# qinzheng93/GeoTransformer

Hardware: NVIDIA H100
Metric: point-cloud pairs/sec (3DMatch-shape synth) (higher is better)
Workload: dtype f32

## Files before the change

geotransformer_b200/_lib.py:

```python
import ctypes
import os
import threading

import torch

_HERE = os.path.dirname(os.path.abspath(__file__))
LIB_PATH = os.path.join(_HERE, 'libgeob200.so')
_lib = None

c_void_p, c_int64, c_int32, c_float, c_double, c_size_t, c_int = (
    ctypes.c_void_p, ctypes.c_int64, ctypes.c_int32, ctypes.c_float, ctypes.c_double, ctypes.c_size_t, ctypes.c_int)

SIGNATURES = {}


def _sig(name, restype, *argtypes):
    SIGNATURES[name] = (restype, list(argtypes))


P, I64, I32, F, D, SZ = c_void_p, c_int64, c_int32, c_float, c_double, c_size_t
_sig('geob200_last_error', ctypes.c_char_p)
_sig('geob200_launch_count', ctypes.c_uint64)
_sig('geob200_grid_subsample_workspace_bytes', SZ, I64, I64)
_sig('geob200_grid_subsample', c_int, P, I64, P, I64, F, P, P, P, SZ, P)
_sig('geob200_radius_search_workspace_bytes', SZ, I64, I64, I64)
_sig('geob200_radius_search', c_int, P, I64, P, I64, P, P, I64, F, I64, P, P, P, P, SZ, P)

_sig('geob200_neighbor_histogram', c_int, P, I64, I64, I64, I64, P, P)
_sig('geob200_kpconv_workspace_bytes', SZ, I64)
_sig('geob200_kpconv', c_int, P, P, P, P, I64, I64, I64, P, I64, P, P, I64, I64, F, P, P, SZ, P)
_sig('geob200_kpconv_tc_workspace_bytes', SZ, I64, I64, I64)
_sig('geob200_kpconv_tc', c_int, P, P, P, P, I64, I64, I64, P, I64, P, P, I64, I64, F, P, P, SZ, P)
_sig('geob200_set_linear_mode', None, c_int)
_sig('geob200_linear', c_int, P, I64, P, P, P, I64, I64, I64, I64, c_int, P)
_sig('geob200_split_tf32', c_int, P, I64, I64, I64, P, P)
_sig('geob200_linear_batched', c_int, P, I64, I64, P, I64, I64, P, I64, P, I64, I64, I64, I64, I64, I64, c_int, P)
_sig('geob200_group_norm_workspace_bytes', SZ, I64)
_sig('geob200_group_norm', c_int, P, I64, I64, I64, P, P, F, P, c_int, F, P, P, SZ, P)
_sig('geob200_fused_group_norm_workspace_bytes', SZ, I64, I64, I64)
_sig('geob200_linear_group_norm', c_int, P, I64, P, P, I64, I64, I64, I64, P, P, F, P, c_int, F, P, P, P, SZ, P)
_sig('geob200_kpconv_group_norm', c_int, P, P, P, P, I64, I64, I64, P, I64, P, P, I64, I64, F, I64, P, P, F, c_int, F, P, P, P, SZ,
     P, SZ, P)
_sig('geob200_group_norm_batched', c_int, P, I64, I64, I64, P, P, F, P, c_int, F, P, P, SZ, P, I64, P)
_sig('geob200_linear_group_norm_batched', c_int, P, I64, P, P, I64, I64, I64, I64, P, P, F, P, c_int, F, P, P, P, SZ, P, I64, P)
_sig('geob200_maxpool', c_int, P, P, I64, I64, I64, I64, P, P)
_sig('geob200_upsample_concat', c_int, P, P, I64, I64, P, I64, I64, I64, P, P)
_sig('geob200_kpconv_backward_workspace_bytes', SZ, I64, I64, I64, I64, I64)
_sig('geob200_kpconv_backward', c_int, P, P, P, P, I64, I64, I64, P, I64, P, I64, I64, F, P, P, P, P, P, SZ, P)
_sig('geob200_linear_backward_workspace_bytes', SZ, I64, I64, I64, c_int)
_sig('geob200_linear_backward', c_int, P, I64, P, P, I64, I64, I64, P, P, P, P, P, SZ, P)
_sig('geob200_group_norm_backward_batched_workspace_bytes', SZ, I64, I64, I64, I64)
_sig('geob200_group_norm_backward_batched', c_int, P, P, I64, I64, I64, P, F, c_int, F, P, P, P, P, P, P, SZ, P, I64, P)
_sig('geob200_maxpool_backward_batched_workspace_bytes', SZ, I64, I64, I64, I64)
_sig('geob200_maxpool_backward_batched', c_int, P, P, I64, I64, I64, I64, P, I64, P, P, P, P, SZ, P)
_sig('geob200_upsample_concat_backward_workspace_bytes', SZ, I64, I64)
_sig('geob200_upsample_concat_backward', c_int, P, I64, I64, I64, I64, I64, P, P, P, P, SZ, P)
_sig('geob200_point_to_node_partition_batched', c_int, P, P, I64, P, P, I64, P, P, P, P, P, P)
_sig('geob200_gather_rows', c_int, P, I64, I64, P, I64, P, P)
_sig('geob200_knn_partition', c_int, P, I64, P, I64, I64, P, P, P)
_sig('geob200_pairwise_distance', c_int, P, I64, P, I64, I64, c_int, P, P)
_sig('geob200_point_to_node_indices', c_int, P, I64, P, I64, P, P, P)
_sig('geob200_apply_transform', c_int, P, I64, P, P, P)
_sig('geob200_gse_indices_batched', c_int, P, I64, P, F, F, I64, P, P, P)
_sig('geob200_gse_embed_workspace_bytes', SZ, I64, I64)
_sig('geob200_gse_table_bytes', SZ, I64, I64, F, F)
_sig('geob200_gse_table_build', c_int, P, P, P, P, P, I64, I64, F, F, P, SZ, P)
_sig('geob200_gse_embed_table', c_int, P, P, I64, I64, P, SZ, I64, F, F, P, P, P, P, P, P, P)
_sig('geob200_gse_embed_pairs', c_int, P, P, I64, I64, P, P, P, P, P, P, P, P, c_int, P, SZ, P)
_sig('geob200_attention_workspace_bytes', SZ, I64, I64, I64)
_sig('geob200_attention', c_int, P, I64, P, I64, P, I64, P, P, P, I64, I64, I64, I64, P, I64, P, SZ, P)
_sig('geob200_set_attention_tma', c_int, c_int)
_sig('geob200_head_bias', c_int, P, I64, P, I64, I64, I64, P, P)
_sig('geob200_add_layernorm', c_int, P, P, P, P, I64, I64, F, P, P)
_sig('geob200_l2_normalize', c_int, P, I64, I64, P, P)
_sig('geob200_add_layernorm_backward_workspace_bytes', SZ, I64, I64)
_sig('geob200_add_layernorm_backward', c_int, P, P, P, I64, I64, F, P, P, P, P, P, SZ, P)
_sig('geob200_l2_normalize_backward', c_int, P, I64, I64, P, P, P)
_sig('geob200_head_project_backward_workspace_bytes', SZ, I64, I64, I64)
_sig('geob200_head_project_backward', c_int, P, I64, P, P, I64, I64, I64, P, P, P, I64, P, P, P, SZ, P)
_sig('geob200_attention_backward_batched_workspace_bytes', SZ, P, I64, I64)
_sig('geob200_attention_backward_batched', c_int, P, P, I64, I64, I64, I64, I64, I64, I64, I64, I64, I64, P, SZ, P)
_sig('geob200_gse_embed_backward_workspace_bytes', SZ, I64, I64)
_sig('geob200_gse_embed_backward', c_int, P, P, I64, I64, I64, P, SZ, I64, F, F, P, P, P, P, P, P, P, P, P, SZ, P)
_sig('geob200_sinkhorn', c_int, P, P, P, P, I64, I64, I64, F, P, P)
_sig('geob200_sinkhorn_backward_workspace_bytes', SZ, I64, I64, I64)
_sig('geob200_sinkhorn_backward', c_int, P, P, P, P, I64, I64, I64, F, P, P, P, P, SZ, P)
_sig('geob200_superpoint_matching_batched_workspace_bytes', SZ, I64, I64, I64)
_sig('geob200_superpoint_matching_batched', c_int, P, P, I64, P, P, I64, P, I64, c_int, P, P, P, P, SZ, P)
_sig('geob200_gather_patches_batched', c_int, P, I64, I64, P, P, P, P, I64, P, P, P, P, P)
_sig('geob200_patch_scores_batched', c_int, P, P, I64, I64, P, P, P, I64, I64, P, P)
_sig('geob200_patch_scores_backward_batched_workspace_bytes', SZ, I64, I64, I64, I64)
_sig('geob200_patch_scores_backward_batched', c_int, P, P, I64, I64, P, P, P, I64, I64, P, P, P, P, SZ, P)
_sig('geob200_lgr_batched_workspace_bytes', SZ, I64, I64, I64, I64)
_sig('geob200_local_global_registration_batched', c_int, P, P, P, P, P, I64, I64, I64, I64, I64, F, c_int, F, I64, I64, P, P, P, P,
     P, P, I64, P, P, P, P, SZ, P)
_sig('geob200_weighted_procrustes', c_int, P, P, P, I64, I64, F, F, P, P)

_sig('geob200_node_correspondences_batched_workspace_bytes', SZ, I64, I64, I64)
_sig('geob200_node_correspondences_batched', c_int, P, P, P, P, P, P, P, P, I64, P, I64, P, F, P, P, P, P, SZ, P)
_sig('geob200_evaluate_counts', c_int, P, P, I64, P, F, P, P, I64, P, P, P, I64, P, F, P, P, P, I64, c_int, F, F, F, P, P)
_sig('geob200_evaluate_batched', c_int, P, P, P, F, P, P, I64, P, P, P, I64, P, F, P, P, I64, P, I64, P, P, c_int, F, F, F, P, I64,
     P)
_sig('geob200_coarse_matching_loss_batched_workspace_bytes', SZ, I64, I64)
_sig('geob200_coarse_matching_loss_batched', c_int, P, P, I64, I64, P, P, P, P, F, F, F, F, F, F, P, I64, P, SZ, P)
_sig('geob200_fine_matching_loss_batched_workspace_bytes', SZ, I64, I64)
_sig('geob200_fine_matching_loss_batched', c_int, P, P, P, P, P, P, I64, I64, I64, P, D, P, P, I64, P, SZ, P)
_sig('geob200_coarse_matching_loss_backward_batched_workspace_bytes', SZ, I64, I64, I64)
_sig('geob200_coarse_matching_loss_backward_batched', c_int, P, P, I64, I64, P, P, P, P, F, F, F, F, F, F, P, I64, P, P, P, P, SZ, P)
_sig('geob200_fine_matching_loss_backward_batched_workspace_bytes', SZ, I64, I64)
_sig('geob200_fine_matching_loss_backward_batched', c_int, P, P, P, P, P, I64, I64, I64, P, D, P, I64, P, P, P, SZ, P)
_sig('geob200_ransac_correspondences_batched_workspace_bytes', SZ, I64, I64)
_sig('geob200_ransac_correspondences_batched', c_int, P, P, I64, I64, P, F, I64, I64, ctypes.c_uint64, I64, P, P, P, P, P, P, P, P, P, P,
     SZ, P)
_sig('geob200_feature_nn_batched_workspace_bytes', SZ, I64, I64, I64)
_sig('geob200_feature_nn_batched', c_int, P, P, I64, I64, I64, I64, P, P, P, P, P, P, P, SZ, P)
_sig('geob200_feature_corr_indices', c_int, P, P, P, P, I64, I64, I32, P, P, P, P, P)
_sig('geob200_ransac_features_batched_workspace_bytes', SZ, I64, I64, I64, I64, I64)
_sig('geob200_ransac_features_batched', c_int, P, P, P, P, I64, I64, I64, I64, P, P, F, I64, I64, I64, ctypes.c_uint64, I64, P, P, P, P, P,
     P, P, P, P, P, P, P, P, P, SZ, P)
_sig('geob200_correspondence_metrics_batched_workspace_bytes', SZ, I64, I64)
_sig('geob200_correspondence_metrics_batched', c_int, P, P, I64, I64, P, P, I64, F, P, I64, P, SZ, P)
_sig('geob200_corr_order_batched', c_int, P, I64, I64, P, I64, P, P)
_sig('geob200_corr_select_batched', c_int, P, P, P, I64, I64, P, P, I64, I64, P, P, P, P, P)
_sig('geob200_sparse_correspondence_eval_batched_workspace_bytes', SZ, I64, I64, I64)
_sig('geob200_sparse_correspondence_eval_batched', c_int, P, P, I64, P, P, I64, P, I64, I64, I64, P, P, SZ, P)
_sig('geob200_registration_error_batched', c_int, P, I64, P, I64, P, P, I64, c_int, D, D, P, P)
_sig('geob200_weighted_procrustes_counts', c_int, P, P, P, I64, I64, P, F, F, P, P)

_sig('geob200_linear_profile_enable', c_int, c_int)
_sig('geob200_set_split_k', c_int, c_int)
_sig('geob200_set_linear_persistent', c_int, c_int)
_sig('geob200_linear_profile_read', I64, I64, P, P)
_sig('geob200_backbone_workspace_bytes', SZ, P, P)
_sig('geob200_backbone_forward_batched', c_int, P, P, P, P, P, P, P, P, P, P, P, P, SZ, P, SZ, P, I64, P, P)
_sig('geob200_cloud_max_count', c_int, P, I64, I64, I64, I64, P, P, P)
_sig('geob200_transformer_batched_workspace_bytes', SZ, I64, P, I64, I64, I64)
_sig('geob200_transformer_forward_batched', c_int, P, I64, I64, I64, P, I64, P, P, P, P, SZ, P)
_sig('geob200_attention_batched_workspace_bytes', SZ, P, I64, I64)
_sig('geob200_attention_batched', c_int, P, I64, I64, I64, I64, I64, I64, I64, P, SZ, P)


def lib():
    global _lib
    if _lib is None:
        if not os.path.exists(LIB_PATH):
            raise RuntimeError(
                f'{LIB_PATH} not found: build it with `python -c "import __graft_entry__ as g; g.build()"` '
                '(there is no CPU fallback for the geotransformer_b200 ops)')
        handle = ctypes.CDLL(LIB_PATH)
        for name, (restype, argtypes) in SIGNATURES.items():
            fn = getattr(handle, name)
            fn.restype = restype
            fn.argtypes = argtypes
        _lib = handle
    return _lib


def check(rc, what):
    if rc != 0:
        msg = lib().geob200_last_error().decode(errors='replace')
        raise RuntimeError(f'{what} failed ({rc}): {msg}')


_tls = threading.local()


def stream_ptr():
    p = getattr(_tls, 'stream', None)
    if p is not None:
        return p
    return torch.cuda.current_stream().cuda_stream


class stream_scope:

    def __init__(self, ptr):
        self.ptr = ptr

    def __enter__(self):
        self.prev = getattr(_tls, 'stream', None)
        _tls.stream = self.ptr
        return self

    def __exit__(self, *a):
        _tls.stream = self.prev
        return False


def require_cuda(t, name, dtype=None):
    if not t.is_cuda:
        raise RuntimeError(f'{name} must be a CUDA tensor (geotransformer_b200 has no CPU path)')
    if dtype is not None and t.dtype != dtype:
        raise RuntimeError(f'{name} must be {dtype}, got {t.dtype}')
    if not t.is_contiguous():
        raise RuntimeError(f'{name} must be contiguous')


_WS = {}


def workspace(nbytes, device, tag='default'):
    key = (device.index if device.index is not None else torch.cuda.current_device(), stream_ptr(), tag)
    buf = _WS.get(key)
    if buf is None or buf.numel() < nbytes:
        buf = torch.empty(max(int(nbytes * 1.3), 1 << 20), dtype=torch.uint8, device=device)
        _WS[key] = buf
    return buf


def ptr(t):
    return None if t is None else t.data_ptr()
```

geotransformer_b200/csrc/attention.cu:

```cuda
#include "attention.cuh"
#include "common.cuh"
#include "geob200.h"

namespace geob200 {

static bool g_att_tma = true;

constexpr int ATT_R = 2;
constexpr int ATT_KPT = 2;
constexpr int ATT_MAXH = 8;
constexpr int ATT_KQ = 8;

template <int H>
__global__ void __launch_bounds__(256) attention_kernel(const float* __restrict__ q, int ldq, const float* __restrict__ k, int ldk,
                                                        const float* __restrict__ v, int ldv, const float* __restrict__ qp,
                                                        const float* __restrict__ qb, const float* __restrict__ E, int N, int M,
                                                        int C, float div, float* __restrict__ out, int ldo) {
    extern __shared__ float sm[];
    float* q_s = sm;
    float* qp_s = q_s + ATT_R * C;
    float* sc = qp_s + ATT_R * H * C;
    const int n0 = blockIdx.x * ATT_R;
    const int lane = threadIdx.x & 31, warp = threadIdx.x >> 5;
    const int d = C / H;
    for (int t = threadIdx.x; t < ATT_R * C; t += blockDim.x) {
        const int r = t / C, n = n0 + r;
        q_s[t] = (n < N) ? q[(long long)n * ldq + (t % C)] : 0.f;
    }
    if (qp != nullptr)
        for (int t = threadIdx.x; t < ATT_R * H * C; t += blockDim.x) {
            const int r = t / (H * C), n = n0 + r;
            qp_s[t] = (n < N) ? qp[(long long)n * H * C + (t % (H * C))] : 0.f;
        }
    __syncthreads();
    const bool has_e = (E != nullptr);
    const int r1ok = (n0 + 1 < N) ? 1 : 0;
    for (int mb = warp * 32 * ATT_KPT; mb < M; mb += 8 * 32 * ATT_KPT) {
        int mk[ATT_KPT];
        bool ok[ATT_KPT];
#pragma unroll
        for (int u = 0; u < ATT_KPT; ++u) { mk[u] = mb + u * 32 + lane; ok[u] = mk[u] < M; if (!ok[u]) mk[u] = M - 1; }
        float tot[ATT_KPT][ATT_R][H];
#pragma unroll
        for (int h = 0; h < H; ++h) {
            float aq[ATT_KPT][ATT_R];
#pragma unroll
            for (int u = 0; u < ATT_KPT; ++u) { aq[u][0] = 0.f; aq[u][1] = 0.f; }
            for (int c = h * d; c < (h + 1) * d; c += 4) {
                const float4 q0 = *reinterpret_cast<const float4*>(q_s + c);
                const float4 q1 = *reinterpret_cast<const float4*>(q_s + C + c);
#pragma unroll
                for (int u = 0; u < ATT_KPT; ++u) {
                    const float4 kv = *reinterpret_cast<const float4*>(k + (long long)mk[u] * ldk + c);
                    aq[u][0] = fmaf(kv.x, q0.x, fmaf(kv.y, q0.y, fmaf(kv.z, q0.z, fmaf(kv.w, q0.w, aq[u][0]))));
                    aq[u][1] = fmaf(kv.x, q1.x, fmaf(kv.y, q1.y, fmaf(kv.z, q1.z, fmaf(kv.w, q1.w, aq[u][1]))));
                }
            }
#pragma unroll
            for (int u = 0; u < ATT_KPT; ++u) { tot[u][0][h] = aq[u][0]; tot[u][1][h] = aq[u][1]; }
        }
        if (has_e) {
            float ae[ATT_KPT][ATT_R][H];
#pragma unroll
            for (int u = 0; u < ATT_KPT; ++u)
#pragma unroll
                for (int r = 0; r < ATT_R; ++r)
#pragma unroll
                    for (int h = 0; h < H; ++h) ae[u][r][h] = 0.f;
            const float* e00 = E + ((long long)n0 * M + mk[0]) * C;
            const float* e01 = E + ((long long)n0 * M + mk[1]) * C;
            const float* e10 = E + ((long long)(n0 + r1ok) * M + mk[0]) * C;
            const float* e11 = E + ((long long)(n0 + r1ok) * M + mk[1]) * C;
#pragma unroll 2
            for (int c = 0; c < C; c += 4) {
                const float4 x00 = __ldg(reinterpret_cast<const float4*>(e00 + c));
                const float4 x01 = __ldg(reinterpret_cast<const float4*>(e01 + c));
                const float4 x10 = __ldg(reinterpret_cast<const float4*>(e10 + c));
                const float4 x11 = __ldg(reinterpret_cast<const float4*>(e11 + c));
#pragma unroll
                for (int h = 0; h < H; ++h) {
                    const float4 a0 = *reinterpret_cast<const float4*>(qp_s + (0 * H + h) * C + c);
                    const float4 a1 = *reinterpret_cast<const float4*>(qp_s + (1 * H + h) * C + c);
                    ae[0][0][h] = fmaf(x00.x, a0.x, fmaf(x00.y, a0.y, fmaf(x00.z, a0.z, fmaf(x00.w, a0.w, ae[0][0][h]))));
                    ae[1][0][h] = fmaf(x01.x, a0.x, fmaf(x01.y, a0.y, fmaf(x01.z, a0.z, fmaf(x01.w, a0.w, ae[1][0][h]))));
                    ae[0][1][h] = fmaf(x10.x, a1.x, fmaf(x10.y, a1.y, fmaf(x10.z, a1.z, fmaf(x10.w, a1.w, ae[0][1][h]))));
                    ae[1][1][h] = fmaf(x11.x, a1.x, fmaf(x11.y, a1.y, fmaf(x11.z, a1.z, fmaf(x11.w, a1.w, ae[1][1][h]))));
                }
            }
#pragma unroll
            for (int u = 0; u < ATT_KPT; ++u)
#pragma unroll
                for (int r = 0; r < ATT_R; ++r)
#pragma unroll
                    for (int h = 0; h < H; ++h)
                        if (n0 + r < N) tot[u][r][h] += ae[u][r][h] + qb[(long long)(n0 + r) * H + h];
        }
#pragma unroll
        for (int u = 0; u < ATT_KPT; ++u)
            if (ok[u]) {
#pragma unroll
                for (int r = 0; r < ATT_R; ++r)
#pragma unroll
                    for (int h = 0; h < H; ++h) sc[(r * H + h) * M + mk[u]] = tot[u][r][h] / div;
            }
    }
    __syncthreads();
    for (int rh = warp; rh < ATT_R * H; rh += 8) {
        float* s = sc + rh * M;
        float mx = -INFINITY;
        for (int m = lane; m < M; m += 32) mx = fmaxf(mx, s[m]);
        mx = warp_max(mx);
        float sum = 0.f;
        for (int m = lane; m < M; m += 32) {
            const float e = expf(s[m] - mx);
            s[m] = e;
            sum += e;
        }
        sum = warp_sum(sum);
        for (int m = lane; m < M; m += 32) s[m] = s[m] / sum;
    }
    __syncthreads();
    for (int c = threadIdx.x; c < C; c += blockDim.x) {
        const int h = c / d;
        const float* p0 = sc + (0 * H + h) * M;
        const float* p1 = sc + (1 * H + h) * M;
        float a0[4] = {0.f, 0.f, 0.f, 0.f}, a1[4] = {0.f, 0.f, 0.f, 0.f};
        int m = 0;
        for (; m + 3 < M; m += 4) {
#pragma unroll
            for (int u = 0; u < 4; ++u) {
                const float vv = v[(long long)(m + u) * ldv + c];
                a0[u] = fmaf(p0[m + u], vv, a0[u]);
                a1[u] = fmaf(p1[m + u], vv, a1[u]);
            }
        }
        for (; m < M; ++m) {
            const float vv = v[(long long)m * ldv + c];
            a0[0] = fmaf(p0[m], vv, a0[0]);
            a1[0] = fmaf(p1[m], vv, a1[0]);
        }
        if (n0 < N) out[(long long)n0 * ldo + c] = (a0[0] + a0[1]) + (a0[2] + a0[3]);
        if (n0 + 1 < N) out[(long long)(n0 + 1) * ldo + c] = (a1[0] + a1[1]) + (a1[2] + a1[3]);
    }
}

constexpr int ATS_G = 4;

__device__ __forceinline__ float dot4(const float4 a, const float4 b, float acc) {
    return fmaf(a.x, b.x, fmaf(a.y, b.y, fmaf(a.z, b.z, fmaf(a.w, b.w, acc))));
}

constexpr int ATS_DEPTH = 3;

__device__ __forceinline__ void cp_async16(void* smem_dst, const void* gsrc) {
    asm volatile("cp.async.cg.shared.global [%0], [%1], 16;" ::"r"((uint32_t)__cvta_generic_to_shared(smem_dst)), "l"(gsrc) : "memory");
}
__device__ __forceinline__ void cp_async_commit() { asm volatile("cp.async.commit_group;" ::: "memory"); }
template <int N>
__device__ __forceinline__ void cp_async_wait() { asm volatile("cp.async.wait_group %0;" ::"n"(N) : "memory"); }

template <int H, int J>
__global__ void __launch_bounds__(128) att_scores_kernel(const __grid_constant__ AttBatch b, int ldq, int ldk, float div) {
    constexpr int C = 128 * J;
    constexpr int D = C / H;
    constexpr int NV = ATS_G * H;
    extern __shared__ float4 ring_all[];
    const int lane = threadIdx.x & 31, warp = threadIdx.x >> 5;
    float4* ring = ring_all + (size_t)warp * ATS_DEPTH * ATS_G * J * 32;
    const bool has_e = (b.it[0].E != nullptr);
    const long long groups = b.gprefix[b.n_items];
    const long long g_begin = groups * blockIdx.x / gridDim.x, g_end = groups * (blockIdx.x + 1) / gridDim.x;
    float4 qv[J];
    float4 qpv[H][J];
    int hq[J];
#pragma unroll
    for (int j = 0; j < J; ++j) hq[j] = (j * 128 + 4 * lane) / D;
    int cp = 0, ci = 0;

    auto prefetch = [&](long long g, int slot) {
        if (has_e && g < g_end) {
            while (g >= b.gprefix[cp + 1]) ++cp;
            const int M = b.it[cp].M;
            const int gpq = (M + ATS_G - 1) / ATS_G;
            const long long gl = g - b.gprefix[cp];
            const int n = (int)(gl / gpq), m0 = (int)(gl % gpq) * ATS_G;
            const float* e_row = b.it[cp].E + (long long)n * M * C;
#pragma unroll
            for (int u = 0; u < ATS_G; ++u) {
                const int m = min(m0 + u, M - 1);
#pragma unroll
                for (int j = 0; j < J; ++j)
                    cp_async16(&ring[((slot * ATS_G + u) * J + j) * 32 + lane], e_row + (long long)m * C + j * 128 + 4 * lane);
            }
        }
        cp_async_commit();
    };

    const long long first = g_begin + warp;
#pragma unroll
    for (int d = 0; d < ATS_DEPTH - 1; ++d) prefetch(first + 4ll * d, d);
    long long n_loaded = -1;
    int slot = 0;
    for (long long g = first; g < g_end; g += 4) {
        prefetch(g + 4ll * (ATS_DEPTH - 1), (slot + ATS_DEPTH - 1) % ATS_DEPTH);
        while (g >= b.gprefix[ci + 1]) ++ci;
        const int M = b.it[ci].M;
        const int gpq = (M + ATS_G - 1) / ATS_G;
        const long long gl = g - b.gprefix[ci];
        const int n = (int)(gl / gpq), m0 = (int)(gl % gpq) * ATS_G;
        const float* __restrict__ k = b.it[ci].k;
        if ((((long long)ci << 32) | n) != n_loaded) {
            const float* __restrict__ q = b.it[ci].q;
            const float* __restrict__ qp = b.it[ci].qp;
#pragma unroll
            for (int j = 0; j < J; ++j) {
                const int c = j * 128 + 4 * lane;
                qv[j] = *reinterpret_cast<const float4*>(q + (long long)n * ldq + c);
#pragma unroll
                for (int h = 0; h < H; ++h)
                    qpv[h][j] = has_e ? *reinterpret_cast<const float4*>(qp + ((long long)n * H + h) * C + c) : make_float4(0.f, 0.f, 0.f, 0.f);
            }
            n_loaded = ((long long)ci << 32) | n;
        }
        float4 kk[ATS_G][J];
#pragma unroll
        for (int u = 0; u < ATS_G; ++u) {
            const int m = min(m0 + u, M - 1);
#pragma unroll
            for (int j = 0; j < J; ++j) kk[u][j] = __ldg(reinterpret_cast<const float4*>(k + (long long)m * ldk + j * 128 + 4 * lane));
        }
        cp_async_wait<ATS_DEPTH - 1>();
        float v[NV];
#pragma unroll
        for (int u = 0; u < ATS_G; ++u) {
#pragma unroll
            for (int h = 0; h < H; ++h) {
                float a = 0.f;
#pragma unroll
                for (int j = 0; j < J; ++j) {
                    const float p = dot4(kk[u][j], qv[j], 0.f);
                    a += (hq[j] == h) ? p : 0.f;
                    if (has_e) a = dot4(ring[((slot * ATS_G + u) * J + j) * 32 + lane], qpv[h][j], a);
                }
                v[u * H + h] = a;
            }
        }
        warp_butterfly(v, lane);
        constexpr int SH = (NV == 32) ? 0 : (NV == 16) ? 1 : (NV == 8) ? 2 : 3;
        const int idx = lane >> SH;
        const int u = idx / H, h = idx % H;
        if ((lane & ((1 << SH) - 1)) == 0 && m0 + u < M) {
            const float bias = has_e ? b.it[ci].qb[(long long)n * H + h] : 0.f;
            b.it[ci].S[((long long)n * H + h) * M + m0 + u] = (v[0] + bias) / div;
        }
        slot = (slot + 1) % ATS_DEPTH;
    }
    cp_async_wait<0>();
}

template <int H>
__global__ void __launch_bounds__(512) att_softmax_pv_kernel(const __grid_constant__ AttBatch b, int ldv, int C, int ldo) {
    extern __shared__ float sm[];
    float* sc = sm;
    const AttItem& item = b.it[blockIdx.y];
    const int N = item.N, M = item.M;
    const int n0 = blockIdx.x * ATT_R;
    if (n0 >= N) return;
    const float* S = item.S;
    const float* __restrict__ v = item.v;
    float* __restrict__ out = item.out;
    const int lane = threadIdx.x & 31, warp = threadIdx.x >> 5;
    const int d = C / H;
    for (int rh = warp; rh < ATT_R * H; rh += (int)(blockDim.x >> 5)) {
        const int r = rh / H;
        float* s = sc + rh * M;
        if (n0 + r >= N) {
            for (int m = lane; m < M; m += 32) s[m] = 0.f;
            continue;
        }
        const float* src = S + ((long long)(n0 + r) * H + (rh % H)) * M;
        float mx = -INFINITY;
        for (int m = lane; m < M; m += 32) { const float x = src[m]; s[m] = x; mx = fmaxf(mx, x); }
        mx = warp_max(mx);
        float sum = 0.f;
        for (int m = lane; m < M; m += 32) {
            const float e = expf(s[m] - mx);
            s[m] = e;
            sum += e;
        }
        sum = warp_sum(sum);
        float* dst = item.S + ((long long)(n0 + r) * H + (rh % H)) * M;
        for (int m = lane; m < M; m += 32) {
            s[m] = s[m] / sum;
            dst[m] = s[m];
        }
    }
    __syncthreads();
    float4* red = reinterpret_cast<float4*>(sc + ((ATT_R * H * M + 3) & ~3));
    const int C4 = C >> 2;
    const int kq = threadIdx.x / 64, c4 = threadIdx.x % 64;
    if (c4 < C4) {
        const int h = (4 * c4) / d;
        const float* p0 = sc + (0 * H + h) * M;
        const float* p1 = sc + (1 * H + h) * M;
        const int per = (M + ATT_KQ - 1) / ATT_KQ, mb = kq * per, me = min(M, mb + per);
        float4 a0 = make_float4(0.f, 0.f, 0.f, 0.f), a1 = a0, b0 = a0, b1 = a0;
        int m = mb;
        for (; m + 3 < me; m += 4) {
            float4 vv[4];
#pragma unroll
            for (int u = 0; u < 4; ++u) vv[u] = __ldg(reinterpret_cast<const float4*>(v + (long long)(m + u) * ldv) + c4);
#pragma unroll
            for (int u = 0; u < 4; u += 2) {
                const float w0 = p0[m + u], w1 = p1[m + u], x0 = p0[m + u + 1], x1 = p1[m + u + 1];
                a0.x = fmaf(w0, vv[u].x, a0.x); a0.y = fmaf(w0, vv[u].y, a0.y); a0.z = fmaf(w0, vv[u].z, a0.z); a0.w = fmaf(w0, vv[u].w, a0.w);
                a1.x = fmaf(w1, vv[u].x, a1.x); a1.y = fmaf(w1, vv[u].y, a1.y); a1.z = fmaf(w1, vv[u].z, a1.z); a1.w = fmaf(w1, vv[u].w, a1.w);
                b0.x = fmaf(x0, vv[u + 1].x, b0.x); b0.y = fmaf(x0, vv[u + 1].y, b0.y); b0.z = fmaf(x0, vv[u + 1].z, b0.z); b0.w = fmaf(x0, vv[u + 1].w, b0.w);
                b1.x = fmaf(x1, vv[u + 1].x, b1.x); b1.y = fmaf(x1, vv[u + 1].y, b1.y); b1.z = fmaf(x1, vv[u + 1].z, b1.z); b1.w = fmaf(x1, vv[u + 1].w, b1.w);
            }
        }
        for (; m < me; ++m) {
            const float4 vv = __ldg(reinterpret_cast<const float4*>(v + (long long)m * ldv) + c4);
            const float w0 = p0[m], w1 = p1[m];
            a0.x = fmaf(w0, vv.x, a0.x); a0.y = fmaf(w0, vv.y, a0.y); a0.z = fmaf(w0, vv.z, a0.z); a0.w = fmaf(w0, vv.w, a0.w);
            a1.x = fmaf(w1, vv.x, a1.x); a1.y = fmaf(w1, vv.y, a1.y); a1.z = fmaf(w1, vv.z, a1.z); a1.w = fmaf(w1, vv.w, a1.w);
        }
        red[(kq * ATT_R + 0) * C4 + c4] = make_float4(a0.x + b0.x, a0.y + b0.y, a0.z + b0.z, a0.w + b0.w);
        red[(kq * ATT_R + 1) * C4 + c4] = make_float4(a1.x + b1.x, a1.y + b1.y, a1.z + b1.z, a1.w + b1.w);
    }
    __syncthreads();
    for (int t = threadIdx.x; t < ATT_R * C4; t += blockDim.x) {
        const int r = t / C4, cc = t % C4;
        if (n0 + r >= N) continue;
        float4 acc = red[(0 * ATT_R + r) * C4 + cc];
#pragma unroll
        for (int g = 1; g < ATT_KQ; ++g) {
            const float4 x = red[(g * ATT_R + r) * C4 + cc];
            acc.x += x.x; acc.y += x.y; acc.z += x.z; acc.w += x.w;
        }
        float* o = out + (long long)(n0 + r) * ldo + 4 * cc;
        o[0] = acc.x; o[1] = acc.y; o[2] = acc.z; o[3] = acc.w;
    }
}

template <int H, int J>
static int launch_streaming(const AttBatch& b, int ldq, int ldk, int ldv, float div, int ldo, cudaStream_t st) {
    constexpr int ring_bytes = 4 * ATS_DEPTH * ATS_G * J * 32 * (int)sizeof(float4);
    if (ring_bytes > 48 * 1024 && ensure_max_smem((const void*)att_scores_kernel<H, J>)) return -1;
    static int per_sm = 0;
    if (per_sm == 0) {
        if (cudaOccupancyMaxActiveBlocksPerMultiprocessor(&per_sm, att_scores_kernel<H, J>, 128, ring_bytes) != cudaSuccess || per_sm < 1)
            per_sm = 1;
    }
    const long long groups = b.gprefix[b.n_items];
    long long grid = (long long)per_sm * num_sms();
    if (grid * 4 > groups) grid = (groups + 3) / 4;
    att_scores_kernel<H, J><<<(unsigned)grid, 128, ring_bytes, st>>>(b, ldq, ldk, div);
    int max_n = 0, max_m = 0;
    for (int i = 0; i < b.n_items; ++i) { max_n = b.it[i].N > max_n ? b.it[i].N : max_n; max_m = b.it[i].M > max_m ? b.it[i].M : max_m; }
    const size_t smem = sizeof(float) * (ATT_R * H * (size_t)((max_m + 3) / 4 * 4) + ATT_KQ * ATT_R * 128 * J);
    if (smem > 48 * 1024 && ensure_max_smem((const void*)att_softmax_pv_kernel<H>)) return -1;
    const dim3 pv_grid((unsigned)((max_n + ATT_R - 1) / ATT_R), (unsigned)b.n_items);
    att_softmax_pv_kernel<H><<<pv_grid, 64 * ATT_KQ, smem, st>>>(b, ldv, 128 * J, ldo);
    return 0;
}

__global__ void __launch_bounds__(256) head_bias_kernel(const float* __restrict__ q, int ldq, const float* __restrict__ bp, int N, int C,
                                                        int H, float* __restrict__ qb) {
    const int t = blockIdx.x * blockDim.x + threadIdx.x;
    if (t >= N * H) return;
    const int n = t / H, h = t % H, d = C / H;
    float s = 0.f;
    for (int c = 0; c < d; ++c) s = fmaf(q[(long long)n * ldq + h * d + c], bp[h * d + c], s);
    qb[t] = s;
}

__global__ void __launch_bounds__(256) add_layernorm_kernel(const float* __restrict__ a, const float* __restrict__ b,
                                                            const float* __restrict__ gamma, const float* __restrict__ beta,
                                                            int N, int C, float eps, float* __restrict__ y) {
    const int lane = threadIdx.x & 31;
    const int n = blockIdx.x * 8 + (threadIdx.x >> 5);
    if (n >= N) return;
    float vals[32];
    float s = 0.f;
    int cnt = 0;
    for (int c = lane; c < C; c += 32, ++cnt) {
        const float x = a[(long long)n * C + c] + (b != nullptr ? b[(long long)n * C + c] : 0.f);
        vals[cnt] = x;
        s += x;
    }
    const float mean = warp_sum(s) / (float)C;
    float s2 = 0.f;
    for (int i = 0; i < cnt; ++i) { const float d = vals[i] - mean; s2 = fmaf(d, d, s2); }
    const float rstd = rsqrtf(warp_sum(s2) / (float)C + eps);
    cnt = 0;
    for (int c = lane; c < C; c += 32, ++cnt) y[(long long)n * C + c] = (vals[cnt] - mean) * rstd * gamma[c] + beta[c];
}

__global__ void __launch_bounds__(256) l2_normalize_kernel(const float* __restrict__ x, int N, int C, float* __restrict__ y) {
    const int lane = threadIdx.x & 31;
    const int n = blockIdx.x * 8 + (threadIdx.x >> 5);
    if (n >= N) return;
    float s = 0.f;
    for (int c = lane; c < C; c += 32) { const float v = x[(long long)n * C + c]; s = fmaf(v, v, s); }
    const float nrm = fmaxf(sqrtf(warp_sum(s)), 1e-12f);
    for (int c = lane; c < C; c += 32) y[(long long)n * C + c] = x[(long long)n * C + c] / nrm;
}

}

using namespace geob200;

extern "C" {

size_t geob200_attention_workspace_bytes(int64_t n_query, int64_t n_key, int64_t heads) {
    return (size_t)n_query * (size_t)n_key * (size_t)heads * sizeof(float) + 256;
}

static int attention_streaming_batch(const geob200_att_item_t* items, int64_t n_items, int64_t ldq, int64_t ldk, int64_t ldv, int64_t ldo,
                                     int64_t channels, int64_t heads, void* workspace, size_t workspace_bytes, cudaStream_t st) {
    if (!(channels == 128 || channels == 256) || workspace == nullptr) return 1;
    GEOB_REQUIRE(n_items >= 1 && n_items <= ATT_MAX_ITEMS, "attention: 1..%d items per launch", ATT_MAX_ITEMS);
    AttBatch b{};
    b.n_items = (int)n_items;
    b.gprefix[0] = 0;
    b.uprefix[0] = 0;
    size_t need = 0;
    for (int i = 0; i < (int)n_items; ++i) {
        const geob200_att_item_t& it = items[i];
        GEOB_REQUIRE(it.n_query > 0 && it.n_key > 0, "attention: empty input");
        GEOB_REQUIRE((it.embed == nullptr) == (it.qp == nullptr) && (it.embed == nullptr) == (it.qb == nullptr), "attention: qp/qb/embed must come together");
        GEOB_REQUIRE((it.embed == nullptr) == (items[0].embed == nullptr), "attention: a batch is all self- or all cross-attention");
        GEOB_REQUIRE(((uintptr_t)it.q % 16) == 0 && ((uintptr_t)it.k % 16) == 0 && ((uintptr_t)it.v % 16) == 0 &&
                         (it.qp == nullptr || ((uintptr_t)it.qp % 16) == 0) && (it.embed == nullptr || ((uintptr_t)it.embed % 16) == 0),
                     "attention: q, k, v, qp, embed must be 16-byte aligned");
        const size_t smem_pv = sizeof(float) * (ATT_R * heads * (size_t)((it.n_key + 3) / 4 * 4) + ATT_KQ * ATT_R * channels);
        if (smem_pv > 200 * 1024) return 1;
        AttItem& d = b.it[i];
        d.q = it.q; d.k = it.k; d.v = it.v; d.qp = it.qp; d.qb = it.qb; d.E = it.embed; d.out = it.out;
        d.N = (int)it.n_query; d.M = (int)it.n_key;
        d.S = (float*)((char*)workspace + need);
        need += align_up((size_t)it.n_query * (size_t)it.n_key * (size_t)heads * sizeof(float), 256);
        b.gprefix[i + 1] = b.gprefix[i] + (long long)it.n_query * ((it.n_key + ATS_G - 1) / ATS_G);
        b.uprefix[i + 1] = b.uprefix[i] + (long long)it.n_query;
    }
    GEOB_REQUIRE(workspace_bytes >= need, "attention: workspace too small");
    const float div = sqrtf((float)(channels / heads));
    if (g_att_tma) {
        const int rt = attention_tma_batch(b, (int)ldq, (int)ldk, (int)ldv, (int)ldo, (int)channels, (int)heads, div, st);
        if (rt <= 0) return rt;
    }
    int rc = -2;
#define LAUNCH_STREAM(HV)                                                                                             \
    rc = (channels == 256) ? launch_streaming<HV, 2>(b, (int)ldq, (int)ldk, (int)ldv, div, (int)ldo, st)              \
                           : launch_streaming<HV, 1>(b, (int)ldq, (int)ldk, (int)ldv, div, (int)ldo, st)
    switch (heads) {
        case 1: LAUNCH_STREAM(1); break;
        case 2: LAUNCH_STREAM(2); break;
        case 4: LAUNCH_STREAM(4); break;
        default: LAUNCH_STREAM(8); break;
    }
#undef LAUNCH_STREAM
    GEOB_REQUIRE(rc == 0, "attention: could not configure the softmax kernel");
    GEOB_CHECK_LAUNCH();
    count_launches(2);
    return 0;
}

static int attention_check(int64_t channels, int64_t heads, int64_t ldq, int64_t ldk, int64_t ldv) {
    GEOB_REQUIRE(channels % 4 == 0 && channels <= 256 && heads > 0 && heads <= ATT_MAXH && channels % heads == 0 &&
                     (channels / heads) % 4 == 0,
                 "attention: unsupported channels=%lld heads=%lld", (long long)channels, (long long)heads);
    GEOB_REQUIRE(ldq % 4 == 0 && ldk % 4 == 0 && ldv % 4 == 0, "attention: row strides must be multiples of 4 floats");
    GEOB_REQUIRE(heads == 1 || heads == 2 || heads == 4 || heads == 8, "attention: heads must be 1, 2, 4 or 8");
    return 0;
}

int geob200_set_attention_tma(int on) {
    g_att_tma = on != 0;
    return 0;
}

size_t geob200_attention_batched_workspace_bytes(const geob200_att_item_t* items, int64_t n_items, int64_t heads) {
    size_t need = 256;
    for (int64_t i = 0; i < n_items; ++i)
        need += align_up((size_t)items[i].n_query * (size_t)items[i].n_key * (size_t)heads * sizeof(float), 256);
    return need;
}

int geob200_attention_batched(const geob200_att_item_t* items, int64_t n_items, int64_t ldq, int64_t ldk, int64_t ldv, int64_t ldo,
                              int64_t channels, int64_t heads, void* workspace, size_t workspace_bytes, void* stream) {
    cudaStream_t st = (cudaStream_t)stream;
    if (n_items == 0) return 0;
    if (attention_check(channels, heads, ldq, ldk, ldv)) return -2;
    for (int64_t i0 = 0; i0 < n_items; i0 += ATT_MAX_ITEMS) {
        const int64_t cnt = (n_items - i0 < ATT_MAX_ITEMS) ? n_items - i0 : ATT_MAX_ITEMS;
        const int rc = attention_streaming_batch(items + i0, cnt, ldq, ldk, ldv, ldo, channels, heads, workspace, workspace_bytes, st);
        if (rc < 0) return rc;
        if (rc == 1)
            for (int64_t i = i0; i < i0 + cnt; ++i) {
                const geob200_att_item_t& it = items[i];
                const int r2 = geob200_attention(it.q, ldq, it.k, ldk, it.v, ldv, it.qp, it.qb, it.embed, it.n_query, it.n_key, channels, heads,
                                                 it.out, ldo, nullptr, 0, stream);
                if (r2 != 0) return r2;
            }
    }
    return 0;
}

int geob200_attention(const float* q, int64_t ldq, const float* k, int64_t ldk, const float* v, int64_t ldv, const float* qp,
                      const float* qb, const float* embed, int64_t n_query, int64_t n_key, int64_t channels, int64_t heads,
                      float* out, int64_t ldo, void* workspace, size_t workspace_bytes, void* stream) {
    cudaStream_t st = (cudaStream_t)stream;
    GEOB_REQUIRE(n_query > 0 && n_key > 0, "attention: empty input");
    if (attention_check(channels, heads, ldq, ldk, ldv)) return -2;
    GEOB_REQUIRE((embed == nullptr) == (qp == nullptr) && (embed == nullptr) == (qb == nullptr), "attention: qp/qb/embed must come together");
    const float div = sqrtf((float)(channels / heads));
    if (workspace != nullptr) {
        const geob200_att_item_t one{q, k, v, qp, qb, embed, out, n_query, n_key};
        const int rc = attention_streaming_batch(&one, 1, ldq, ldk, ldv, ldo, channels, heads, workspace, workspace_bytes, st);
        if (rc <= 0) return rc;
    }
    const size_t smem = sizeof(float) * (ATT_R * channels + ATT_R * heads * channels + ATT_R * heads * n_key);
    GEOB_REQUIRE(smem <= 200 * 1024, "attention: too many keys (%lld)", (long long)n_key);
    if (smem > 48 * 1024 && (ensure_max_smem((const void*)attention_kernel<1>) || ensure_max_smem((const void*)attention_kernel<2>) ||
                             ensure_max_smem((const void*)attention_kernel<4>) || ensure_max_smem((const void*)attention_kernel<8>))) return -1;
    const unsigned grid = (unsigned)((n_query + ATT_R - 1) / ATT_R);
#define LAUNCH_ATT(HV)                                                                                                              \
    attention_kernel<HV><<<grid, 256, smem, st>>>(q, (int)ldq, k, (int)ldk, v, (int)ldv, qp, qb, embed, (int)n_query, (int)n_key,  \
                                                  (int)channels, div, out, (int)ldo)
    switch (heads) {
        case 1: LAUNCH_ATT(1); break;
        case 2: LAUNCH_ATT(2); break;
        case 4: LAUNCH_ATT(4); break;
        default: LAUNCH_ATT(8); break;
    }
#undef LAUNCH_ATT
    GEOB_CHECK_LAUNCH();
    count_launches(1);
    return 0;
}

int geob200_head_bias(const float* q, int64_t ldq, const float* bias_p, int64_t n, int64_t channels, int64_t heads, float* qb,
                      void* stream) {
    head_bias_kernel<<<(unsigned)((n * heads + 255) / 256), 256, 0, (cudaStream_t)stream>>>(q, (int)ldq, bias_p, (int)n, (int)channels,
                                                                                          (int)heads, qb);
    GEOB_CHECK_LAUNCH();
    count_launches(1);
    return 0;
}

int geob200_add_layernorm(const float* a, const float* b, const float* gamma, const float* beta, int64_t n, int64_t channels,
                          float eps, float* y, void* stream) {
    GEOB_REQUIRE(channels <= 1024, "add_layernorm: channels > 1024");
    add_layernorm_kernel<<<(unsigned)((n + 7) / 8), 256, 0, (cudaStream_t)stream>>>(a, b, gamma, beta, (int)n, (int)channels, eps, y);
    GEOB_CHECK_LAUNCH();
    count_launches(1);
    return 0;
}

int geob200_l2_normalize(const float* x, int64_t n, int64_t channels, float* y, void* stream) {
    l2_normalize_kernel<<<(unsigned)((n + 7) / 8), 256, 0, (cudaStream_t)stream>>>(x, (int)n, (int)channels, y);
    GEOB_CHECK_LAUNCH();
    count_launches(1);
    return 0;
}

}
```

geotransformer_b200/csrc/attention.cuh:

```cuda
#pragma once
#include <cuda_runtime.h>

namespace geob200 {

constexpr int ATT_MAX_ITEMS = 32;
struct AttItem { const float *q, *k, *v, *qp, *qb, *E; float *out, *S; int N, M; };
struct AttBatch {
    int n_items;
    int reserved;
    long long gprefix[ATT_MAX_ITEMS + 1];
    long long uprefix[ATT_MAX_ITEMS + 1];
    AttItem it[ATT_MAX_ITEMS];
};

int attention_tma_batch(const AttBatch& b, int ldq, int ldk, int ldv, int ldo, int channels, int heads, float div, cudaStream_t st);

}
```

geotransformer_b200/csrc/attention_tma.cu:

```cuda
#include "attention.cuh"
#include "common.cuh"
#include "geob200.h"

namespace geob200 {

__device__ __forceinline__ uint32_t at_smem_u32(const void* p) { return (uint32_t)__cvta_generic_to_shared(p); }
__device__ __forceinline__ void at_mbar_init(uint64_t* bar, uint32_t count) {
    asm volatile("mbarrier.init.shared::cta.b64 [%0], %1;" ::"r"(at_smem_u32(bar)), "r"(count));
}
__device__ __forceinline__ void at_mbar_arrive(uint64_t* bar) {
    asm volatile("{\n\t.reg .b64 st;\n\tmbarrier.arrive.shared::cta.b64 st, [%0];\n\t}" ::"r"(at_smem_u32(bar)) : "memory");
}
__device__ __forceinline__ void at_mbar_arrive_expect_tx(uint64_t* bar, uint32_t bytes) {
    asm volatile("{\n\t.reg .b64 st;\n\tmbarrier.arrive.expect_tx.shared::cta.b64 st, [%0], %1;\n\t}" ::"r"(at_smem_u32(bar)), "r"(bytes)
                 : "memory");
}
__device__ __forceinline__ void at_mbar_wait(uint64_t* bar, uint32_t parity) {
    const uint32_t addr = at_smem_u32(bar);
    uint32_t done;
    do {
        asm volatile("{\n\t.reg .pred p;\n\tmbarrier.try_wait.parity.shared::cta.b64 p, [%1], %2;\n\tselp.u32 %0, 1, 0, p;\n\t}"
                     : "=r"(done)
                     : "r"(addr), "r"(parity)
                     : "memory");
    } while (!done);
}
__device__ __forceinline__ void at_bulk_g2s(void* dst, const void* src, uint32_t bytes, uint64_t* bar) {
    asm volatile("cp.async.bulk.shared::cluster.global.mbarrier::complete_tx::bytes [%0], [%1], %2, [%3];" ::"r"(at_smem_u32(dst)),
                 "l"(src), "r"(bytes), "r"(at_smem_u32(bar))
                 : "memory");
}

constexpr int ATQ_T = 64;
constexpr int ATQ_LD = ATQ_T + 4;

template <int H>
__global__ void __launch_bounds__(256) att_qk_kernel(const __grid_constant__ AttBatch b, int ldq, int ldk, int D) {
    __shared__ __align__(16) float Qs[32][ATQ_LD], Ks[32][ATQ_LD];
    const int item = blockIdx.z / H, h = blockIdx.z % H;
    const AttItem& it = b.it[item];
    const int N = it.N, M = it.M;
    const int n0 = blockIdx.y * ATQ_T, m0 = blockIdx.x * ATQ_T;
    if (n0 >= N || m0 >= M) return;
    const int tx = threadIdx.x & 15, ty = threadIdx.x >> 4;
    float acc[4][4];
#pragma unroll
    for (int i = 0; i < 4; ++i)
#pragma unroll
        for (int j = 0; j < 4; ++j) acc[i][j] = 0.f;
    for (int d0 = 0; d0 < D; d0 += 32) {
        const int dd = threadIdx.x & 31, r8 = threadIdx.x >> 5;
#pragma unroll
        for (int i = 0; i < 8; ++i) {
            const int r = r8 + 8 * i;
            Qs[dd][r] = (n0 + r < N && d0 + dd < D) ? it.q[(long long)(n0 + r) * ldq + h * D + d0 + dd] : 0.f;
            Ks[dd][r] = (m0 + r < M && d0 + dd < D) ? it.k[(long long)(m0 + r) * ldk + h * D + d0 + dd] : 0.f;
        }
        __syncthreads();
#pragma unroll 8
        for (int d = 0; d < 32; ++d) {
            const float4 qv = *reinterpret_cast<const float4*>(&Qs[d][4 * ty]);
            const float4 kv = *reinterpret_cast<const float4*>(&Ks[d][4 * tx]);
            const float qa[4] = {qv.x, qv.y, qv.z, qv.w}, ka[4] = {kv.x, kv.y, kv.z, kv.w};
#pragma unroll
            for (int i = 0; i < 4; ++i)
#pragma unroll
                for (int j = 0; j < 4; ++j) acc[i][j] = fmaf(qa[i], ka[j], acc[i][j]);
        }
        __syncthreads();
    }
#pragma unroll
    for (int i = 0; i < 4; ++i) {
        const int n = n0 + 4 * ty + i;
        if (n >= N) continue;
        float* row = it.S + ((long long)n * H + h) * M + m0 + 4 * tx;
#pragma unroll
        for (int j = 0; j < 4; ++j)
            if (m0 + 4 * tx + j < M) row[j] = acc[i][j];
    }
}

constexpr int ATM_KCH = 16;
constexpr int ATM_NST = 4;
constexpr int ATM_CW = 8;
constexpr int ATM_THREADS = (ATM_CW + 1) * 32;

template <int H, int J>
__global__ void __launch_bounds__(ATM_THREADS) att_stream_kernel(const __grid_constant__ AttBatch b, float div, int max_m) {
    constexpr int C = 128 * J;
    constexpr int NV = 2 * H;
    static_assert(NV == 2 || NV == 4 || NV == 8 || NV == 16, "heads must be 1, 2, 4 or 8");
    extern __shared__ unsigned char atm_smem_raw[];
    unsigned char* smem = (unsigned char*)(((uintptr_t)atm_smem_raw + 127) & ~(uintptr_t)127);
    float4* ring = reinterpret_cast<float4*>(smem);
    float* sc = reinterpret_cast<float*>(smem + (size_t)ATM_NST * ATM_KCH * C * 4);
    const int mp = (max_m + 3) & ~3;
    uint64_t* full = reinterpret_cast<uint64_t*>(sc + (size_t)H * mp);
    uint64_t* empty = full + ATM_NST;
    const int warp = threadIdx.x >> 5, lane = threadIdx.x & 31;
    if (threadIdx.x == 0) {
        for (int s = 0; s < ATM_NST; ++s) { at_mbar_init(&full[s], 1); at_mbar_init(&empty[s], ATM_CW); }
        asm volatile("fence.mbarrier_init.release.cluster;" ::: "memory");
    }
    __syncthreads();
    const long long units = b.uprefix[b.n_items];
    const long long u_begin = units * blockIdx.x / gridDim.x, u_end = units * (blockIdx.x + 1) / gridDim.x;

    if (warp == ATM_CW) {
        if (lane == 0) {
            int s = 0, ci = 0;
            uint32_t ph = 0;
            for (long long u = u_begin; u < u_end; ++u) {
                while (u >= b.uprefix[ci + 1]) ++ci;
                const int M = b.it[ci].M;
                const int n = (int)(u - b.uprefix[ci]);
                const float* e_row = b.it[ci].E + (long long)n * M * C;
                for (int m0 = 0; m0 < M; m0 += ATM_KCH) {
                    const uint32_t bytes = (uint32_t)(min(ATM_KCH, M - m0) * C * 4);
                    at_mbar_wait(&empty[s], ph ^ 1u);
                    at_mbar_arrive_expect_tx(&full[s], bytes);
                    at_bulk_g2s(ring + (size_t)s * ATM_KCH * (C / 4), e_row + (long long)m0 * C, bytes, &full[s]);
                    if (++s == ATM_NST) { s = 0; ph ^= 1u; }
                }
            }
        }
        return;
    }

    int s = 0, ci = 0;
    uint32_t ph = 0;
    for (long long u = u_begin; u < u_end; ++u) {
        while (u >= b.uprefix[ci + 1]) ++ci;
        const AttItem& it = b.it[ci];
        const int M = it.M;
        const int n = (int)(u - b.uprefix[ci]);
        float4 qpv[H][J];
#pragma unroll
        for (int h = 0; h < H; ++h)
#pragma unroll
            for (int j = 0; j < J; ++j)
                qpv[h][j] = *reinterpret_cast<const float4*>(it.qp + ((long long)n * H + h) * C + j * 128 + 4 * lane);
        constexpr int SH = (NV == 16) ? 1 : (NV == 8) ? 2 : (NV == 4) ? 3 : 4;
        const int vidx = lane >> SH, vu = vidx / H, vh = vidx % H;
        const float qb_h = it.qb[(long long)n * H + vh];
        float* S_row = it.S + ((long long)n * H + vh) * M;
        for (int m0 = 0; m0 < M; m0 += ATM_KCH) {
            const int mk = m0 + 2 * warp + vu;
            const bool writer = (lane & ((1 << SH) - 1)) == 0 && mk < M && (2 * warp + vu) < ATM_KCH;
            const float sqk = writer ? S_row[mk] : 0.f;
            at_mbar_wait(&full[s], ph);
            const float4* st = ring + (size_t)s * ATM_KCH * (C / 4);
            float v[NV];
#pragma unroll
            for (int uu = 0; uu < 2; ++uu) {
                const int kk = 2 * warp + uu;
#pragma unroll
                for (int h = 0; h < H; ++h) v[uu * H + h] = 0.f;
#pragma unroll
                for (int j = 0; j < J; ++j) {
                    const float4 e = st[(size_t)kk * (C / 4) + j * 32 + lane];
#pragma unroll
                    for (int h = 0; h < H; ++h)
                        v[uu * H + h] = fmaf(e.x, qpv[h][j].x, fmaf(e.y, qpv[h][j].y, fmaf(e.z, qpv[h][j].z, fmaf(e.w, qpv[h][j].w, v[uu * H + h]))));
                }
            }
            __syncwarp();
            if (lane == 0) at_mbar_arrive(&empty[s]);
            if (++s == ATM_NST) { s = 0; ph ^= 1u; }
            warp_butterfly(v, lane);
            if (writer) sc[vh * mp + mk] = (sqk + v[0] + qb_h) / div;
        }
        asm volatile("bar.sync 1, %0;" ::"n"(ATM_CW * 32) : "memory");
        for (int h = warp; h < H; h += ATM_CW) {
            float* sh = sc + h * mp;
            float mx = -INFINITY;
            for (int m = lane; m < M; m += 32) mx = fmaxf(mx, sh[m]);
            mx = warp_max(mx);
            float sum = 0.f;
            for (int m = lane; m < M; m += 32) {
                const float e = expf(sh[m] - mx);
                sh[m] = e;
                sum += e;
            }
            sum = warp_sum(sum);
            float* dst = it.S + ((long long)n * H + h) * M;
            for (int m = lane; m < M; m += 32) dst[m] = sh[m] / sum;
        }
        asm volatile("bar.sync 1, %0;" ::"n"(ATM_CW * 32) : "memory");
    }
}

template <int H>
__global__ void __launch_bounds__(256) att_pv_kernel(const __grid_constant__ AttBatch b, int ldv, int ldo, int D) {
    __shared__ __align__(16) float Ps[32][ATQ_LD], Vs[32][ATQ_LD];
    const AttItem& it = b.it[blockIdx.z];
    const int dtiles = (D + 63) / 64;
    const int h = blockIdx.y / dtiles, d0 = (blockIdx.y % dtiles) * 64;
    const int N = it.N, M = it.M;
    const int n0 = blockIdx.x * ATQ_T;
    if (n0 >= N) return;
    const int tx = threadIdx.x & 15, ty = threadIdx.x >> 4;
    float acc[4][4];
#pragma unroll
    for (int i = 0; i < 4; ++i)
#pragma unroll
        for (int j = 0; j < 4; ++j) acc[i][j] = 0.f;
    for (int m0 = 0; m0 < M; m0 += 32) {
        {
            const int km = threadIdx.x & 31, r8 = threadIdx.x >> 5;
#pragma unroll
            for (int i = 0; i < 8; ++i) {
                const int r = r8 + 8 * i;
                Ps[km][r] = (n0 + r < N && m0 + km < M) ? it.S[((long long)(n0 + r) * H + h) * M + m0 + km] : 0.f;
            }
            const int dc = threadIdx.x & 63, r4 = threadIdx.x >> 6;
#pragma unroll
            for (int i = 0; i < 8; ++i) {
                const int r = r4 + 4 * i;
                Vs[r][dc] = (m0 + r < M && d0 + dc < D) ? it.v[(long long)(m0 + r) * ldv + h * D + d0 + dc] : 0.f;
            }
        }
        __syncthreads();
#pragma unroll 8
        for (int mm = 0; mm < 32; ++mm) {
            const float4 pv = *reinterpret_cast<const float4*>(&Ps[mm][4 * ty]);
            const float4 vv = *reinterpret_cast<const float4*>(&Vs[mm][4 * tx]);
            const float pa[4] = {pv.x, pv.y, pv.z, pv.w}, va[4] = {vv.x, vv.y, vv.z, vv.w};
#pragma unroll
            for (int i = 0; i < 4; ++i)
#pragma unroll
                for (int j = 0; j < 4; ++j) acc[i][j] = fmaf(pa[i], va[j], acc[i][j]);
        }
        __syncthreads();
    }
#pragma unroll
    for (int i = 0; i < 4; ++i) {
        const int n = n0 + 4 * ty + i;
        if (n >= N) continue;
        float* row = it.out + (long long)n * ldo + h * D + d0 + 4 * tx;
#pragma unroll
        for (int j = 0; j < 4; ++j)
            if (d0 + 4 * tx + j < D) row[j] = acc[i][j];
    }
}

template <int H>
__global__ void __launch_bounds__(256) att_softmax_kernel(const __grid_constant__ AttBatch b, float div) {
    const int lane = threadIdx.x & 31;
    const long long row = (long long)blockIdx.x * 8 + (threadIdx.x >> 5);
    if (row >= b.uprefix[b.n_items] * H) return;
    const long long u = row / H;
    int ci = 0;
    while (u >= b.uprefix[ci + 1]) ++ci;
    const AttItem& it = b.it[ci];
    const int M = it.M;
    float* s = it.S + ((u - b.uprefix[ci]) * H + (row % H)) * M;
    float mx = -INFINITY;
    for (int m = lane; m < M; m += 32) mx = fmaxf(mx, s[m] / div);
    mx = warp_max(mx);
    float sum = 0.f;
    for (int m = lane; m < M; m += 32) {
        const float e = expf(s[m] / div - mx);
        s[m] = e;
        sum += e;
    }
    sum = warp_sum(sum);
    for (int m = lane; m < M; m += 32) s[m] = s[m] / sum;
}

template <int H>
static int launch_cross(const AttBatch& b, int ldq, int ldk, int ldv, int ldo, int D, float div, cudaStream_t st) {
    int max_n = 0, max_m = 0;
    for (int i = 0; i < b.n_items; ++i) { max_n = b.it[i].N > max_n ? b.it[i].N : max_n; max_m = b.it[i].M > max_m ? b.it[i].M : max_m; }
    const dim3 qk_grid((unsigned)((max_m + ATQ_T - 1) / ATQ_T), (unsigned)((max_n + ATQ_T - 1) / ATQ_T), (unsigned)(b.n_items * H));
    att_qk_kernel<H><<<qk_grid, 256, 0, st>>>(b, ldq, ldk, D);
    const long long rows = b.uprefix[b.n_items] * H;
    att_softmax_kernel<H><<<(unsigned)((rows + 7) / 8), 256, 0, st>>>(b, div);
    const dim3 pv_grid((unsigned)((max_n + ATQ_T - 1) / ATQ_T), (unsigned)(H * ((D + 63) / 64)), (unsigned)b.n_items);
    att_pv_kernel<H><<<pv_grid, 256, 0, st>>>(b, ldv, ldo, D);
    return 0;
}

template <int H, int J>
static int launch_tma(const AttBatch& b, int ldq, int ldk, int ldv, int ldo, float div, cudaStream_t st) {
    constexpr int C = 128 * J, D = C / H;
    int max_n = 0, max_m = 0;
    for (int i = 0; i < b.n_items; ++i) { max_n = b.it[i].N > max_n ? b.it[i].N : max_n; max_m = b.it[i].M > max_m ? b.it[i].M : max_m; }
    const dim3 qk_grid((unsigned)((max_m + ATQ_T - 1) / ATQ_T), (unsigned)((max_n + ATQ_T - 1) / ATQ_T), (unsigned)(b.n_items * H));
    att_qk_kernel<H><<<qk_grid, 256, 0, st>>>(b, ldq, ldk, D);
    const size_t smem = (size_t)ATM_NST * ATM_KCH * C * 4 + sizeof(float) * H * (size_t)((max_m + 3) & ~3) + 2 * ATM_NST * 8 + 256;
    if (ensure_max_smem((const void*)att_stream_kernel<H, J>)) return -1;
    int occ = 0;
    if (cudaOccupancyMaxActiveBlocksPerMultiprocessor(&occ, att_stream_kernel<H, J>, ATM_THREADS, smem) != cudaSuccess || occ < 1) occ = 1;
    const long long units = b.uprefix[b.n_items];
    long long grid = (long long)occ * num_sms();
    if (grid > units) grid = units;
    att_stream_kernel<H, J><<<(unsigned)grid, ATM_THREADS, smem, st>>>(b, div, max_m);
    const dim3 pv_grid((unsigned)((max_n + ATQ_T - 1) / ATQ_T), (unsigned)(H * ((D + 63) / 64)), (unsigned)b.n_items);
    att_pv_kernel<H><<<pv_grid, 256, 0, st>>>(b, ldv, ldo, D);
    return 0;
}

int attention_tma_batch(const AttBatch& b, int ldq, int ldk, int ldv, int ldo, int channels, int heads, float div, cudaStream_t st) {
    if (b.it[0].E == nullptr) {
        int rc = -2;
        switch (heads) {
            case 1: rc = launch_cross<1>(b, ldq, ldk, ldv, ldo, channels / heads, div, st); break;
            case 2: rc = launch_cross<2>(b, ldq, ldk, ldv, ldo, channels / heads, div, st); break;
            case 4: rc = launch_cross<4>(b, ldq, ldk, ldv, ldo, channels / heads, div, st); break;
            case 8: rc = launch_cross<8>(b, ldq, ldk, ldv, ldo, channels / heads, div, st); break;
            default: return 1;
        }
        if (rc != 0) return rc;
        GEOB_CHECK_LAUNCH();
        count_launches(3);
        return 0;
    }
    if (!(channels == 128 || channels == 256)) return 1;
    int max_m = 0;
    for (int i = 0; i < b.n_items; ++i) max_m = b.it[i].M > max_m ? b.it[i].M : max_m;
    const size_t smem = (size_t)ATM_NST * ATM_KCH * channels * 4 + sizeof(float) * heads * (size_t)((max_m + 3) & ~3) + 2 * ATM_NST * 8 + 256;
    if (smem > 200 * 1024) return 1;
    int rc = -2;
#define LAUNCH_TMA(HV) rc = (channels == 256) ? launch_tma<HV, 2>(b, ldq, ldk, ldv, ldo, div, st) : launch_tma<HV, 1>(b, ldq, ldk, ldv, ldo, div, st)
    switch (heads) {
        case 1: LAUNCH_TMA(1); break;
        case 2: LAUNCH_TMA(2); break;
        case 4: LAUNCH_TMA(4); break;
        case 8: LAUNCH_TMA(8); break;
        default: return 1;
    }
#undef LAUNCH_TMA
    if (rc != 0) return rc;
    GEOB_CHECK_LAUNCH();
    count_launches(3);
    return 0;
}

}
```

geotransformer_b200/csrc/gse_table.cu:

```cuda
#include "common.cuh"
#include "geob200.h"
#include "gse_table.cuh"

namespace geob200 {
namespace gtab {

template <int C>
__global__ void __launch_bounds__(C) table_scale_kernel(const float* __restrict__ div_term, const float* __restrict__ WdT,
                                                        const float* __restrict__ WaT, int inv_step, int n_d, int n_a,
                                                        Header* __restrict__ hdr) {
    __shared__ float red[C / 32];
    const int c = threadIdx.x;
    float bd = 0.f, ba = 0.f;
    for (int k = 0; k < C; ++k) {
        const float f = div_term[k >> 1];
        bd = fmaf(f, fabsf(WdT[(size_t)k * C + c]), bd);
        ba = fmaf(f, fabsf(WaT[(size_t)k * C + c]), ba);
    }
    float b = warp_max(fmaxf(bd, ba) / (float)inv_step);
    if ((c & 31) == 0) red[c >> 5] = b;
    __syncthreads();
    if (c == 0) {
        for (int w = 1; w < C / 32; ++w) b = fmaxf(b, red[w]);
        int e = 14;
        if (b > 0.f && b < 3.0e38f) (void)frexpf(b, &e);
        e = max(-100, min(100, e - 14));
        hdr->magic = MAGIC;
        hdr->channels = C;
        hdr->inv_step = inv_step;
        hdr->n_d = n_d;
        hdr->n_a = n_a;
        hdr->slope_scale = ldexpf(1.0f, e);
        hdr->inv_slope_scale = ldexpf(1.0f, -e);
    }
}

template <int C>
__global__ void __launch_bounds__(C) table_build_kernel(const float* __restrict__ div_term, const float* __restrict__ WdT,
                                                        const float* __restrict__ WaT, const float* __restrict__ bd,
                                                        const float* __restrict__ ba, int inv_step, int n_d,
                                                        unsigned char* __restrict__ table) {
    __shared__ double s0[C], s1[C];
    const Header* hdr = reinterpret_cast<const Header*>(table);
    const int node = blockIdx.x;
    const bool angle = node >= n_d;
    const int i = angle ? node - n_d : node;
    const float* __restrict__ WT = angle ? WaT : WdT;
    const float* __restrict__ bias = angle ? ba : bd;
    const double h = 1.0 / (double)inv_step;
    const double x0 = (double)i * h, x1 = x0 + h;
    const int t = threadIdx.x;
    if (t < C / 2) {
        const double f = (double)div_term[t];
        double s, c;
        sincos(x0 * f, &s, &c);
        s0[2 * t] = s;
        s0[2 * t + 1] = c;
        sincos(x1 * f, &s, &c);
        s1[2 * t] = s;
        s1[2 * t + 1] = c;
    }
    __syncthreads();
    double a0 = 0.0, a1 = 0.0;
    for (int k = 0; k < C; ++k) {
        const double w = (double)WT[(size_t)k * C + t];
        a0 = fma(w, s0[k], a0);
        a1 = fma(w, s1[k], a1);
    }
    unsigned char* nodep = table + HEADER_BYTES + (size_t)node * (C * 6);
    reinterpret_cast<float*>(nodep)[t] = (float)(a0 + (double)bias[t]);
    reinterpret_cast<__half*>(nodep + C * 4)[t] = __float2half_rn((float)((a1 - a0) * (double)hdr->inv_slope_scale));
}

template <int C>
__global__ void __launch_bounds__(256, 4) table_embed_kernel(const float* __restrict__ d_idx, const float* __restrict__ a_idx,
                                                             long long n_pairs, const unsigned char* __restrict__ table, int n_d,
                                                             int n_a, float inv_step, const float* __restrict__ div_term,
                                                             const float* __restrict__ Wd, const float* __restrict__ Wa,
                                                             const float* __restrict__ bd, const float* __restrict__ ba,
                                                             float* __restrict__ E) {
    using LK = Lookup<C>;
    constexpr int NV = LK::NV;
    __shared__ float4 idx_s[8][32];
    const int lane = threadIdx.x & 31, warp = threadIdx.x >> 5;
    const float scale = reinterpret_cast<const Header*>(table)->slope_scale;
    const unsigned char* __restrict__ td = table + HEADER_BYTES;
    const unsigned char* __restrict__ ta = td + (size_t)n_d * LK::NODE;
    const float lim_d = (float)n_d, lim_a = (float)n_a;
    const long long n_chunks = (n_pairs + 31) / 32;
    for (long long chunk = (long long)blockIdx.x * 8 + warp; chunk < n_chunks; chunk += (long long)gridDim.x * 8) {
        const long long p0 = chunk * 32;
        const long long p = p0 + lane;
        float4 v = make_float4(0.f, 0.f, 0.f, 0.f);
        if (p < n_pairs) {
            v.x = d_idx[p];
            v.y = a_idx[3 * p];
            v.z = a_idx[3 * p + 1];
            v.w = a_idx[3 * p + 2];
        }
        __syncwarp();
        idx_s[warp][lane] = v;
        __syncwarp();
        const long long left = n_pairs - p0;
        const int cnt = left < 32 ? (int)left : 32;
        for (int r = 0; r < cnt; ++r) {
            const float4 x = idx_s[warp][r];
            const float t0 = x.x * inv_step, t1 = x.y * inv_step, t2 = x.z * inv_step, t3 = x.w * inv_step;
            const bool in0 = t0 >= 0.f && t0 < lim_d, in1 = t1 >= 0.f && t1 < lim_a, in2 = t2 >= 0.f && t2 < lim_a,
                       in3 = t3 >= 0.f && t3 < lim_a;
            float* __restrict__ row = E + (p0 + r) * C;
            if (!(in0 && in1 && in2 && in3)) {
                LK::slow_row(x, td, ta, lim_d, lim_a, inv_step, scale, div_term, Wd, Wa, bd, ba, lane, row);
                continue;
            }
            float vd[4 * NV], va[4 * NV], vb[4 * NV], vc[4 * NV];
            const int i0 = (int)t0, i1 = (int)t1, i2 = (int)t2, i3 = (int)t3;
            LK::interp(td, i0, (t0 - (float)i0) * scale, lane, vd);
            LK::interp(ta, i1, (t1 - (float)i1) * scale, lane, va);
            LK::interp(ta, i2, (t2 - (float)i2) * scale, lane, vb);
            LK::interp(ta, i3, (t3 - (float)i3) * scale, lane, vc);
#pragma unroll
            for (int j = 0; j < NV; ++j) {
                float4 o;
                o.x = vd[4 * j + 0] + fmaxf(fmaxf(va[4 * j + 0], vb[4 * j + 0]), vc[4 * j + 0]);
                o.y = vd[4 * j + 1] + fmaxf(fmaxf(va[4 * j + 1], vb[4 * j + 1]), vc[4 * j + 1]);
                o.z = vd[4 * j + 2] + fmaxf(fmaxf(va[4 * j + 2], vb[4 * j + 2]), vc[4 * j + 2]);
                o.w = vd[4 * j + 3] + fmaxf(fmaxf(va[4 * j + 3], vb[4 * j + 3]), vc[4 * j + 3]);
                __stcs(reinterpret_cast<float4*>(row) + 32 * j + lane, o);
            }
        }
    }
}

}
}

using namespace geob200;

static int table_grid(long long n_pairs) {
    const long long chunks = (n_pairs + 31) / 32;
    const long long ctas = (chunks + 7) / 8;
    const long long full = (long long)num_sms() * 4;
    return (int)(ctas < full ? ctas : full);
}

extern "C" {

size_t geob200_gse_table_bytes(int64_t channels, int64_t inv_step, float d_max, float a_max) {
    if (channels <= 0 || inv_step <= 0 || !(d_max > 0.f) || !(a_max > 0.f)) return 0;
    const size_t nodes = (size_t)gtab::node_count(d_max, (int)inv_step) + (size_t)gtab::node_count(a_max, (int)inv_step);
    return gtab::HEADER_BYTES + nodes * (size_t)channels * 6;
}

int geob200_gse_table_build(const float* div_term, const float* wd_t, const float* wa_t, const float* bd, const float* ba,
                            int64_t channels, int64_t inv_step, float d_max, float a_max, void* table, size_t table_bytes,
                            void* stream) {
    cudaStream_t st = (cudaStream_t)stream;
    GEOB_REQUIRE(channels == 128 || channels == 256, "gse_table_build: channels %lld unsupported (128 or 256)", (long long)channels);
    GEOB_REQUIRE(inv_step >= 1 && inv_step <= 65536 && (inv_step & (inv_step - 1)) == 0,
                 "gse_table_build: inv_step %lld must be a power of two", (long long)inv_step);
    GEOB_REQUIRE(d_max > 0.f && a_max > 0.f && (double)d_max * inv_step < 1.6e7 && (double)a_max * inv_step < 1.6e7,
                 "gse_table_build: bad range");
    GEOB_REQUIRE(table_bytes >= geob200_gse_table_bytes(channels, inv_step, d_max, a_max), "gse_table_build: table buffer too small");
    GEOB_REQUIRE(((uintptr_t)table & 15) == 0, "gse_table_build: table must be 16-byte aligned");
    const int n_d = gtab::node_count(d_max, (int)inv_step), n_a = gtab::node_count(a_max, (int)inv_step);
    unsigned char* tb = (unsigned char*)table;
    if (channels == 256) {
        gtab::table_scale_kernel<256><<<1, 256, 0, st>>>(div_term, wd_t, wa_t, (int)inv_step, n_d, n_a, (gtab::Header*)tb);
        gtab::table_build_kernel<256><<<(unsigned)(n_d + n_a), 256, 0, st>>>(div_term, wd_t, wa_t, bd, ba, (int)inv_step, n_d, tb);
    } else {
        gtab::table_scale_kernel<128><<<1, 128, 0, st>>>(div_term, wd_t, wa_t, (int)inv_step, n_d, n_a, (gtab::Header*)tb);
        gtab::table_build_kernel<128><<<(unsigned)(n_d + n_a), 128, 0, st>>>(div_term, wd_t, wa_t, bd, ba, (int)inv_step, n_d, tb);
    }
    GEOB_CHECK_LAUNCH();
    count_launches(2);
    return 0;
}

int geob200_gse_embed_table(const float* d_indices, const float* a_indices, int64_t n_rows, int64_t channels, const void* table,
                            size_t table_bytes, int64_t inv_step, float d_max, float a_max, const float* div_term, const float* wd,
                            const float* wa, const float* bd, const float* ba, float* embeddings, void* stream) {
    cudaStream_t st = (cudaStream_t)stream;
    GEOB_REQUIRE(n_rows > 0, "gse_embed_table: bad shape");
    GEOB_REQUIRE(channels == 128 || channels == 256, "gse_embed_table: channels %lld unsupported (128 or 256)", (long long)channels);
    GEOB_REQUIRE(inv_step >= 1 && (inv_step & (inv_step - 1)) == 0, "gse_embed_table: inv_step must be a power of two");
    GEOB_REQUIRE(table_bytes >= geob200_gse_table_bytes(channels, inv_step, d_max, a_max) && table_bytes > 0,
                 "gse_embed_table: table buffer smaller than (channels, inv_step, d_max, a_max) imply");
    GEOB_REQUIRE(((uintptr_t)table & 15) == 0 && ((uintptr_t)embeddings & 15) == 0, "gse_embed_table: table / embeddings must be 16-byte aligned");
    const int n_d = gtab::node_count(d_max, (int)inv_step), n_a = gtab::node_count(a_max, (int)inv_step);
    const int grid = table_grid((long long)n_rows);
    const unsigned char* tb = (const unsigned char*)table;
    if (channels == 256)
        gtab::table_embed_kernel<256><<<grid, 256, 0, st>>>(d_indices, a_indices, (long long)n_rows, tb, n_d, n_a, (float)inv_step, div_term,
                                                            wd, wa, bd, ba, embeddings);
    else
        gtab::table_embed_kernel<128><<<grid, 256, 0, st>>>(d_indices, a_indices, (long long)n_rows, tb, n_d, n_a, (float)inv_step, div_term,
                                                            wd, wa, bd, ba, embeddings);
    GEOB_CHECK_LAUNCH();
    count_launches(1);
    return 0;
}

}
```

geotransformer_b200/csrc/gse_table.cuh:

```cuda
#pragma once
#include <cuda_fp16.h>
#include <math.h>

#include "common.cuh"

namespace geob200 {
namespace gtab {

constexpr int HEADER_BYTES = 256;
constexpr unsigned MAGIC = 0x47534554u;

struct Header {
    unsigned magic;
    int channels;
    int inv_step;
    int n_d;
    int n_a;
    float slope_scale;
    float inv_slope_scale;
};

template <int C>
struct Lookup {
    static constexpr int NV = C / 128;
    static constexpr int NODE = C * 6;

    static __device__ __forceinline__ void exact(float x, const float* __restrict__ div_term, const float* __restrict__ W,
                                                 const float* __restrict__ bias, int lane, float (&val)[4 * NV]) {
#pragma unroll
        for (int q = 0; q < 4 * NV; ++q) val[q] = 0.f;
        for (int f = 0; f < C / 2; ++f) {
            float s, c;
            sincosf(__fmul_rn(x, div_term[f]), &s, &c);
#pragma unroll
            for (int j = 0; j < NV; ++j)
#pragma unroll
                for (int e = 0; e < 4; ++e) {
                    const int ch = 128 * j + 4 * lane + e;
                    const float2 w = *reinterpret_cast<const float2*>(W + (size_t)ch * C + 2 * f);
                    val[4 * j + e] = fmaf(w.y, c, fmaf(w.x, s, val[4 * j + e]));
                }
        }
#pragma unroll
        for (int j = 0; j < NV; ++j)
#pragma unroll
            for (int e = 0; e < 4; ++e) val[4 * j + e] += bias[128 * j + 4 * lane + e];
    }

    static __device__ __forceinline__ void interp(const unsigned char* __restrict__ tab, int i, float fr, int lane, float (&val)[4 * NV]) {
        const unsigned char* node = tab + (size_t)i * NODE;
#pragma unroll
        for (int j = 0; j < NV; ++j) {
            const float4 f = __ldg(reinterpret_cast<const float4*>(node) + 32 * j + lane);
            const uint2 sraw = __ldg(reinterpret_cast<const uint2*>(node + C * 4) + 32 * j + lane);
            const float2 s01 = __half22float2(*reinterpret_cast<const __half2*>(&sraw.x));
            const float2 s23 = __half22float2(*reinterpret_cast<const __half2*>(&sraw.y));
            val[4 * j + 0] = fmaf(fr, s01.x, f.x);
            val[4 * j + 1] = fmaf(fr, s01.y, f.y);
            val[4 * j + 2] = fmaf(fr, s23.x, f.z);
            val[4 * j + 3] = fmaf(fr, s23.y, f.w);
        }
    }

    static __device__ __forceinline__ void term(float x, const unsigned char* __restrict__ tab, float lim, float inv_step, float scale,
                                                const float* __restrict__ div_term, const float* __restrict__ W,
                                                const float* __restrict__ bias, int lane, float (&val)[4 * NV]) {
        const float t = x * inv_step;
        if (t >= 0.f && t < lim) {
            const int i = (int)t;
            interp(tab, i, (t - (float)i) * scale, lane, val);
        } else {
            exact(x, div_term, W, bias, lane, val);
        }
    }

    static __device__ __noinline__ void slow_row(float4 x, const unsigned char* __restrict__ td, const unsigned char* __restrict__ ta,
                                                 float lim_d, float lim_a, float inv_step, float scale, const float* __restrict__ div_term,
                                                 const float* __restrict__ Wd, const float* __restrict__ Wa, const float* __restrict__ bd,
                                                 const float* __restrict__ ba, int lane, float* __restrict__ row) {
        float acc[4 * NV], val[4 * NV];
        term(x.y, ta, lim_a, inv_step, scale, div_term, Wa, ba, lane, acc);
        term(x.z, ta, lim_a, inv_step, scale, div_term, Wa, ba, lane, val);
#pragma unroll
        for (int q = 0; q < 4 * NV; ++q) acc[q] = fmaxf(acc[q], val[q]);
        term(x.w, ta, lim_a, inv_step, scale, div_term, Wa, ba, lane, val);
#pragma unroll
        for (int q = 0; q < 4 * NV; ++q) acc[q] = fmaxf(acc[q], val[q]);
        term(x.x, td, lim_d, inv_step, scale, div_term, Wd, bd, lane, val);
#pragma unroll
        for (int j = 0; j < NV; ++j)
            __stcs(reinterpret_cast<float4*>(row) + 32 * j + lane,
                   make_float4(val[4 * j + 0] + acc[4 * j + 0], val[4 * j + 1] + acc[4 * j + 1], val[4 * j + 2] + acc[4 * j + 2],
                               val[4 * j + 3] + acc[4 * j + 3]));
    }
};

static inline int node_count(double x_max, int inv_step) { return (int)ceil(x_max * (double)inv_step) + 1; }

}
}
```

geotransformer_b200/csrc/native.cu:

```cuda
#include "common.cuh"
#include "geob200.h"

namespace geob200 {

struct Ctx {
    Arena ar;
    void* gn_ws;
    size_t gn_ws_bytes;
    void* stream;
    int groups;
    Ctx(void* p, size_t n) : ar(p, n) {}
    float* fl(int64_t rows, int64_t ch) { return ar.take<float>((size_t)rows * (size_t)ch); }
};

#define TRY(expr)                  \
    do {                           \
        int _rc = (expr);          \
        if (_rc != 0) return _rc;  \
    } while (0)

static int run_kpconv(Ctx& c, const geob200_kpconv_t& k, const float* s_feats, const float* q_pts, const float* s_pts,
                      const int64_t* nbr, int64_t m, int64_t ns, int64_t h, float* out) {
    const bool tc = (k.c_in % 32 == 0) && (k.c_out % 16 == 0) && k.c_out >= 32 && (k.c_out <= 128 || k.c_out % 128 == 0) && m >= 64 &&
                    k.weights_t != nullptr;
    if (tc) {
        const size_t wb = geob200_kpconv_tc_workspace_bytes(m, ns, k.c_in);
        const size_t mark = c.ar.off;
        void* ws = c.ar.take<char>(wb);
        GEOB_REQUIRE(c.ar.ok(), "native: arena too small (kpconv)");
        TRY(kpconv_tc_impl(s_feats, q_pts, s_pts, nbr, m, ns, h, k.kernel_points, 15, k.weights_t, k.weights_img, k.bias, k.c_in, k.c_out,
                           k.sigma, out, ws, wb, c.stream));
        c.ar.off = mark;
        return 0;
    }
    const size_t wb = geob200_kpconv_workspace_bytes(ns);
    const size_t mark = c.ar.off;
    void* ws = c.ar.take<char>(wb);
    GEOB_REQUIRE(c.ar.ok(), "native: arena too small (kpconv)");
    TRY(geob200_kpconv(s_feats, q_pts, s_pts, nbr, m, ns, h, k.kernel_points, 15, k.weights, k.bias, k.c_in, k.c_out, k.sigma, out, ws,
                       wb, c.stream));
    c.ar.off = mark;
    return 0;
}

static int run_kpconv_norm(Ctx& c, const geob200_kpconv_t& k, const geob200_norm_t& n, const float* s_feats, const float* q_pts,
                           const float* s_pts, const int64_t* nbr, int64_t m, int64_t ns, int64_t h, float* out, const GnSeg* seg) {
    float* y = c.fl(m, k.c_out);
    GEOB_REQUIRE(c.ar.ok(), "native: arena too small (kpconv output)");
    const bool tc = (k.c_in % 32 == 0) && (k.c_out % 16 == 0) && k.c_out >= 32 && (k.c_out <= 128 || k.c_out % 128 == 0) && m >= 64 &&
                    k.weights_t != nullptr;
    if (tc) {
        const size_t wb = geob200_kpconv_tc_workspace_bytes(m, ns, k.c_in);
        const size_t mark = c.ar.off;
        void* ws = c.ar.take<char>(wb);
        GEOB_REQUIRE(c.ar.ok(), "native: arena too small (kpconv)");
        TRY(kpconv_group_norm_impl(s_feats, q_pts, s_pts, nbr, m, ns, h, k.kernel_points, 15, k.weights_t, k.bias, k.c_in, k.c_out,
                                   k.sigma, c.groups, n.gamma, n.beta, 1e-5f, 1, 0.1f, y, out, c.gn_ws, c.gn_ws_bytes, ws, wb, c.stream, seg,
                                   k.weights_img));
        c.ar.off = mark;
        return 0;
    }
    TRY(run_kpconv(c, k, s_feats, q_pts, s_pts, nbr, m, ns, h, y));
    return group_norm_impl(y, m, k.c_out, c.groups, n.gamma, n.beta, 1e-5f, nullptr, 1, 0.1f, out, c.gn_ws, c.gn_ws_bytes, c.stream, seg);
}

static int run_unary(Ctx& c, const geob200_linear_t& l, const geob200_norm_t& n, const float* x, int64_t rows, const float* residual,
                     int leaky, float* out, const GnSeg* seg) {
    float* t = c.fl(rows, l.c_out);
    GEOB_REQUIRE(c.ar.ok(), "native: arena too small (unary)");
    TRY(linear_group_norm_impl(x, l.c_in, l.weight, l.bias, rows, l.c_out, l.c_in, c.groups, n.gamma, n.beta, 1e-5f, residual, leaky,
                               0.1f, t, out, c.gn_ws, c.gn_ws_bytes, c.stream, seg, l.weight_img));
    return 0;
}

static int run_resblock(Ctx& c, const geob200_resblock_t& b, const float* feats, int64_t ns, const float* q_pts, const float* s_pts,
                        const int64_t* nbr, int64_t m, int64_t h, float* out, const GnSeg* seg_s, const GnSeg* seg_q,
                        const int* cloud_max = nullptr) {
    const float* x = feats;
    if (b.has_unary1) {
        float* u = c.fl(ns, b.unary1.c_out);
        TRY(run_unary(c, b.unary1, b.norm1, feats, ns, nullptr, 1, u, seg_s));
        x = u;
    }
    float* yn = c.fl(m, b.conv.c_out);
    GEOB_REQUIRE(c.ar.ok(), "native: arena too small (resblock)");
    TRY(run_kpconv_norm(c, b.conv, b.norm_conv, x, q_pts, s_pts, nbr, m, ns, h, yn, seg_q));
    const float* sc = feats;
    if (b.strided) {
        float* mp = c.fl(m, b.c_in);
        GEOB_REQUIRE(c.ar.ok(), "native: arena too small (maxpool)");
        if (seg_q != nullptr && cloud_max != nullptr) {
            TRY(maxpool_seg(feats, nbr, m, ns, h, b.c_in, mp, seg_q, cloud_max, c.stream));
        } else {
            TRY(geob200_maxpool(feats, nbr, m, ns, h, b.c_in, mp, c.stream));
        }
        sc = mp;
    }
    if (b.has_shortcut) {
        float* s2 = c.fl(m, b.shortcut.c_out);
        TRY(run_unary(c, b.shortcut, b.norm_sc, sc, m, nullptr, 0, s2, seg_q));
        sc = s2;
    }
    return run_unary(c, b.unary2, b.norm2, yn, m, sc, 1, out, seg_q);
}

}

using namespace geob200;

extern "C" {

size_t geob200_backbone_workspace_bytes(const geob200_backbone_t* net, const int64_t* level_rows) {
    size_t total = 1 << 20;
    for (int l = 0; l < net->num_stages; ++l) {
        const size_t rows = (size_t)level_rows[l];
        const size_t ch = (size_t)net->init_dim << (l + 1);
        total += rows * ch * 4 * 24;
        total += geob200_kpconv_tc_workspace_bytes(level_rows[l], l > 0 ? level_rows[l - 1] : level_rows[l], (int64_t)(ch / 2)) + 4096;
    }
    return total;
}

int geob200_backbone_forward_batched(const geob200_backbone_t* net, const float* feats, const float* const* points,
                                     const int64_t* level_rows, const int64_t* const* neighbors, const int64_t* neighbor_width,
                                     const int64_t* const* subsampling, const int64_t* subsampling_width,
                                     const int64_t* const* upsampling, const int64_t* upsampling_width, float* const* out_feats,
                                     void* gn_workspace, size_t gn_workspace_bytes, void* workspace, size_t workspace_bytes, void* stream,
                                     int64_t n_pairs, const int64_t* const* cloud_rows_h, const int32_t* const* sub_cloud_max) {
    GEOB_REQUIRE(n_pairs == 1 || sub_cloud_max != nullptr, "backbone: batched execution needs the per-cloud subsampling widths");
    GEOB_REQUIRE(net->num_stages >= 2 && net->num_stages <= GEOB200_MAX_STAGES, "backbone: num_stages out of range");
    GEOB_REQUIRE(n_pairs >= 1 && 2 * n_pairs <= GEOB_MAX_CLOUDS, "backbone: 1 <= pairs per batch <= %d", GEOB_MAX_CLOUDS / 2);
    GEOB_REQUIRE(n_pairs == 1 || cloud_rows_h != nullptr, "backbone: batched execution needs the per-cloud row counts of every level");
    Ctx c(workspace, workspace_bytes);
    c.gn_ws = gn_workspace; c.gn_ws_bytes = gn_workspace_bytes; c.stream = stream; c.groups = net->groups;
    const int S = net->num_stages;
    GnSeg segs[GEOB200_MAX_STAGES];
    const GnSeg* sg[GEOB200_MAX_STAGES];
    for (int l = 0; l < S; ++l) {
        sg[l] = nullptr;
        if (n_pairs > 1) {
            GnSeg& g = segs[l];
            g.n_pairs = (int)n_pairs; g.n_clouds = (int)(2 * n_pairs); g.start[0] = 0;
            for (int cl = 0; cl < g.n_clouds; ++cl) g.start[cl + 1] = g.start[cl] + (int)cloud_rows_h[l][cl];
            GEOB_REQUIRE(g.start[g.n_clouds] == level_rows[l], "backbone: cloud rows of level %d do not add up", l);
            sg[l] = &g;
        }
    }
    const float* enc[GEOB200_MAX_STAGES];
    int64_t enc_ch[GEOB200_MAX_STAGES];
    {
        const int64_t n0 = level_rows[0];
        float* yn = c.fl(n0, net->conv1.c_out);
        GEOB_REQUIRE(c.ar.ok(), "native: arena too small (encoder1_1)");
        TRY(run_kpconv_norm(c, net->conv1, net->norm1, feats, points[0], points[0], neighbors[0], n0, n0, neighbor_width[0], yn, sg[0]));
        const geob200_resblock_t& b = net->blocks[0];
        float* o = c.fl(n0, b.unary2.c_out);
        TRY(run_resblock(c, b, yn, n0, points[0], points[0], neighbors[0], n0, neighbor_width[0], o, sg[0], sg[0]));
        enc[0] = o; enc_ch[0] = b.unary2.c_out;
    }
    int bi = 1;
    for (int lvl = 1; lvl < S; ++lvl) {
        const int64_t m = level_rows[lvl], ns = level_rows[lvl - 1];
        const geob200_resblock_t& b1 = net->blocks[bi++];
        float* o1 = c.fl(m, b1.unary2.c_out);
        TRY(run_resblock(c, b1, enc[lvl - 1], ns, points[lvl], points[lvl - 1], subsampling[lvl - 1], m, subsampling_width[lvl - 1], o1,
                         sg[lvl - 1], sg[lvl], sub_cloud_max != nullptr ? sub_cloud_max[lvl - 1] : nullptr));
        const geob200_resblock_t& b2 = net->blocks[bi++];
        float* o2 = c.fl(m, b2.unary2.c_out);
        TRY(run_resblock(c, b2, o1, m, points[lvl], points[lvl], neighbors[lvl], m, neighbor_width[lvl], o2, sg[lvl], sg[lvl]));
        const geob200_resblock_t& b3 = net->blocks[bi++];
        float* o3 = (lvl == S - 1) ? out_feats[0] : c.fl(m, b3.unary2.c_out);
        TRY(run_resblock(c, b3, o2, m, points[lvl], points[lvl], neighbors[lvl], m, neighbor_width[lvl], o3, sg[lvl], sg[lvl]));
        enc[lvl] = o3; enc_ch[lvl] = b3.unary2.c_out;
    }
    const float* latent = enc[S - 1];
    int64_t latent_ch = enc_ch[S - 1];
    int oi = 1;
    for (int lvl = S - 1; lvl >= net->finest_decoder; --lvl) {
        const int64_t m = level_rows[lvl - 1], ns = level_rows[lvl];
        const int64_t c2 = enc_ch[lvl - 1];
        float* cat = c.fl(m, latent_ch + c2);
        GEOB_REQUIRE(c.ar.ok(), "native: arena too small (decoder)");
        TRY(geob200_upsample_concat(latent, upsampling[lvl - 1], upsampling_width[lvl - 1], ns, enc[lvl - 1], m, latent_ch, c2, cat, stream));
        const geob200_linear_t& l = net->decoders[S - 1 - lvl];
        float* o = out_feats[oi++];
        if (lvl == net->finest_decoder) {
            TRY(linear_img(cat, l.c_in, l.weight, l.weight_img, l.bias, o, l.c_out, m, l.c_out, l.c_in, 0, stream));
        } else {
            TRY(run_unary(c, l, net->decoder_norms[S - 1 - lvl], cat, m, nullptr, 1, o, sg[lvl - 1]));
        }
        latent = o; latent_ch = l.c_out;
    }
    GEOB_REQUIRE(c.ar.ok(), "native: arena too small");
    return 0;
}


static int run_tail(Ctx& c, const geob200_tlayer_t& L, const float* hidden, const float* inp, int64_t rows, int64_t ch, float* out) {
    float* h = c.fl(rows, ch);
    float* x = c.fl(rows, ch);
    float* y1 = c.fl(rows, 2 * ch);
    float* y2 = c.fl(rows, ch);
    GEOB_REQUIRE(c.ar.ok(), "native: arena too small (transformer tail)");
    TRY(linear_img(hidden, ch, L.att_linear.weight, L.att_linear.weight_img, L.att_linear.bias, h, ch, rows, ch, ch, 0, c.stream));
    TRY(geob200_add_layernorm(h, inp, L.att_norm.gamma, L.att_norm.beta, rows, ch, 1e-5f, x, c.stream));
    TRY(linear_img(x, ch, L.expand.weight, L.expand.weight_img, L.expand.bias, y1, 2 * ch, rows, 2 * ch, ch, 1, c.stream));
    TRY(linear_img(y1, 2 * ch, L.squeeze.weight, L.squeeze.weight_img, L.squeeze.bias, y2, ch, rows, ch, 2 * ch, 0, c.stream));
    TRY(geob200_add_layernorm(x, y2, L.out_norm.gamma, L.out_norm.beta, rows, ch, 1e-5f, out, c.stream));
    return 0;
}

size_t geob200_transformer_batched_workspace_bytes(int64_t n_pairs, const int64_t* cloud_rows_h, int64_t channels, int64_t heads,
                                                   int64_t num_layers) {
    size_t n = 0, att = 0;
    for (int64_t c = 0; c < 2 * n_pairs; ++c) {
        n += (size_t)cloud_rows_h[c];
        const size_t other = (size_t)cloud_rows_h[(c + n_pairs) % (2 * n_pairs)];
        const size_t m = (size_t)cloud_rows_h[c] > other ? (size_t)cloud_rows_h[c] : other;
        att += align_up((size_t)cloud_rows_h[c] * m * (size_t)heads * 4, 256);
    }
    return (n * (size_t)channels * 4 * (3 + 1 + (size_t)heads + 12)) * (size_t)(num_layers + 1) + att + (2 << 20);
}

int geob200_transformer_forward_batched(const geob200_tlayer_t* layers, int64_t num_layers, int64_t channels, int64_t heads,
                                        const float* x_in, int64_t n_pairs, const int64_t* cloud_rows_h, const float* const* embeddings,
                                        float* out, void* workspace, size_t workspace_bytes, void* stream) {
    GEOB_REQUIRE(n_pairs >= 1 && 2 * n_pairs <= GEOB_MAX_CLOUDS, "transformer: 1 <= pairs per batch <= %d", GEOB_MAX_CLOUDS / 2);
    Ctx c(workspace, workspace_bytes);
    c.stream = stream;
    const int64_t C = channels, H = heads, B = n_pairs, NC = 2 * n_pairs;
    int64_t off[GEOB_MAX_CLOUDS + 1];
    off[0] = 0;
    for (int64_t i = 0; i < NC; ++i) off[i + 1] = off[i] + cloud_rows_h[i];
    const int64_t n = off[NC], R = off[B];
    const float* x = x_in;
    geob200_att_item_t items[GEOB_MAX_CLOUDS];
    size_t att_ws_bytes = 0;
    {
        for (int64_t i = 0; i < NC; ++i) { items[i].n_query = cloud_rows_h[i]; items[i].n_key = cloud_rows_h[i]; }
        att_ws_bytes = geob200_attention_batched_workspace_bytes(items, NC, H);
        for (int64_t p = 0; p < B; ++p) { items[p].n_query = cloud_rows_h[p]; items[p].n_key = cloud_rows_h[B + p]; }
        const size_t cross = geob200_attention_batched_workspace_bytes(items, B, H);
        if (cross > att_ws_bytes) att_ws_bytes = cross;
    }
    void* att_ws = c.fl((int64_t)(att_ws_bytes / 4 + 1), 1);
    for (int64_t i = 0; i < num_layers; ++i) {
        const geob200_tlayer_t& L = layers[i];
        float* y = (i == num_layers - 1) ? out : c.fl(n, C);
        if (L.is_self) {
            float* qkv = c.fl(n, 3 * C);
            float* qp = c.fl(n, H * C);
            float* qb = c.fl(n, H);
            float* hidden = c.fl(n, C);
            GEOB_REQUIRE(c.ar.ok(), "native: arena too small (self layer)");
            TRY(linear_img(x, C, L.w_qkv, L.w_qkv_img, L.b_qkv, qkv, 3 * C, n, 3 * C, C, 0, stream));
            const int64_t d = C / H;
            TRY(geob200_linear_batched(qkv, 3 * C, d, L.wp_t, C, d, nullptr, 0, qp, H * C, C, n, C, d, H, 0, stream));
            TRY(geob200_head_bias(qkv, 3 * C, L.bp, n, C, H, qb, stream));
            for (int64_t cl = 0; cl < NC; ++cl) {
                const int64_t o = off[cl];
                items[cl] = geob200_att_item_t{qkv + o * 3 * C, qkv + o * 3 * C + C, qkv + o * 3 * C + 2 * C, qp + o * H * C, qb + o * H,
                                               embeddings[cl], hidden + o * C, cloud_rows_h[cl], cloud_rows_h[cl]};
            }
            TRY(geob200_attention_batched(items, NC, 3 * C, 3 * C, 3 * C, C, C, H, att_ws, att_ws_bytes, stream));
            TRY(run_tail(c, L, hidden, x, n, C, y));
        } else {
            const int64_t Sn = n - R;
            float* q0 = c.fl(R, C);
            float* kv1 = c.fl(Sn, 2 * C);
            float* hid0 = c.fl(R, C);
            float* q1 = c.fl(Sn, C);
            float* kv0 = c.fl(R, 2 * C);
            float* hid1 = c.fl(Sn, C);
            GEOB_REQUIRE(c.ar.ok(), "native: arena too small (cross layer)");
            TRY(linear_img(x, C, L.w_q, L.w_q_img, L.b_q, q0, C, R, C, C, 0, stream));
            TRY(linear_img(x + R * C, C, L.w_kv, L.w_kv_img, L.b_kv, kv1, 2 * C, Sn, 2 * C, C, 0, stream));
            for (int64_t p = 0; p < B; ++p) {
                const int64_t ro = off[p], so = off[B + p] - R;
                items[p] = geob200_att_item_t{q0 + ro * C, kv1 + so * 2 * C, kv1 + so * 2 * C + C, nullptr, nullptr, nullptr, hid0 + ro * C,
                                              cloud_rows_h[p], cloud_rows_h[B + p]};
            }
            TRY(geob200_attention_batched(items, B, C, 2 * C, 2 * C, C, C, H, att_ws, att_ws_bytes, stream));
            TRY(run_tail(c, L, hid0, x, R, C, y));
            TRY(linear_img(x + R * C, C, L.w_q, L.w_q_img, L.b_q, q1, C, Sn, C, C, 0, stream));
            TRY(linear_img(y, C, L.w_kv, L.w_kv_img, L.b_kv, kv0, 2 * C, R, 2 * C, C, 0, stream));
            for (int64_t p = 0; p < B; ++p) {
                const int64_t ro = off[p], so = off[B + p] - R;
                items[p] = geob200_att_item_t{q1 + so * C, kv0 + ro * 2 * C, kv0 + ro * 2 * C + C, nullptr, nullptr, nullptr, hid1 + so * C,
                                              cloud_rows_h[B + p], cloud_rows_h[p]};
            }
            TRY(geob200_attention_batched(items, B, C, 2 * C, 2 * C, C, C, H, att_ws, att_ws_bytes, stream));
            TRY(run_tail(c, L, hid1, x + R * C, Sn, C, y + R * C));
        }
        x = y;
    }
    return 0;
}

}
```

geotransformer_b200/model.py:

```python
import torch
import torch.nn as nn

from . import _lib
from . import functional as GF
from .backbone import KPConvFPN
from .modules.geotransformer import GeometricTransformer, SuperPointMatching, LocalGlobalRegistration
from .modules.sinkhorn import LearnableLogOptimalTransport


class GeoTransformer(nn.Module):
    def __init__(self, cfg):
        super().__init__()
        self.cfg = cfg
        self.num_points_in_patch = cfg.model.num_points_in_patch
        self.matching_radius = cfg.model.ground_truth_matching_radius
        self.fine_level = cfg.model.fine_level
        b = cfg.backbone
        self.backbone = KPConvFPN(b.input_dim, b.output_dim, b.init_dim, b.kernel_size, b.init_radius, b.init_sigma,
                                  b.group_norm, num_stages=b.num_stages,
                                  finest_decoder=2 if self.fine_level == 1 else 1)
        g = cfg.geotransformer
        self.transformer = GeometricTransformer(g.input_dim, g.output_dim, g.hidden_dim, g.num_heads, g.blocks, g.sigma_d,
                                                g.sigma_a, g.angle_k, reduction_a=g.reduction_a)
        self.coarse_matching = SuperPointMatching(cfg.coarse_matching.num_correspondences,
                                                  cfg.coarse_matching.dual_normalization)
        f = cfg.fine_matching
        self.fine_matching = LocalGlobalRegistration(
            f.topk, f.acceptance_radius, mutual=f.mutual, confidence_threshold=f.confidence_threshold,
            use_dustbin=f.use_dustbin, use_global_score=f.use_global_score,
            correspondence_threshold=f.correspondence_threshold, correspondence_limit=f.correspondence_limit,
            num_refinement_steps=f.num_refinement_steps)
        self.optimal_transport = LearnableLogOptimalTransport(cfg.model.num_sinkhorn_iterations)

    @torch.no_grad()
    def forward_batch(self, data_dict, evaluator=None, results=None, side_streams=None, keep_outputs=True, loss_func=None, loss_out=None,
                      ransac=None, ransac_out=None, taps=None):
        B = int(data_dict.get('batch_size', 1))
        forced = data_dict.get('forced_node_corr')
        if B > 1 and (taps is not None or forced is not None):
            raise ValueError('forward_batch: taps and forced_node_corr apply to one pair per forward')
        native = getattr(self, '_native', None)
        if native is None and B > 1:
            raise RuntimeError('forward_batch of several pairs needs the native stage drivers: call enable_native(model) first')
        dev = data_dict['features'].device
        if forced is not None:
            forced = _forced_node_corr(forced, dev)
        marks = data_dict.get('_stage_events')

        def mark(label):
            if marks is not None:
                e = torch.cuda.Event(enable_timing=True)
                e.record()
                marks.append((label, e))
        mark('start')
        lens_h = data_dict.get('lengths_host') or [l.tolist() for l in data_dict['lengths']]
        fl, K = self.fine_level, self.num_points_in_patch
        offs = []
        for lv in lens_h:
            o = [0]
            for v in lv:
                o.append(o[-1] + int(v))
            offs.append(o)
        oc, of, o0 = offs[-1], offs[fl], offs[0]
        points_c, points_f, points0 = data_dict['points'][-1], data_dict['points'][fl], data_dict['points'][0]
        cloud = lambda t, o, c: t[o[c]:o[c + 1]]
        main = torch.cuda.current_stream()
        sides = side_streams or [main]
        no_sync = results is not None

        def fork():
            ev = torch.cuda.Event()
            ev.record(main)
            for s in sides:
                if s is not main:
                    s.wait_event(ev)

        def join():
            for s in sides:
                if s is not main:
                    ev = torch.cuda.Event()
                    ev.record(s)
                    main.wait_event(ev)

        class on:
            def __init__(self, i):
                self.s = sides[i % len(sides)]
            def __enter__(self):
                self.a = torch.cuda.stream(self.s); self.a.__enter__()
                self.b = _lib.stream_scope(self.s.cuda_stream); self.b.__enter__()
            def __exit__(self, *e):
                self.b.__exit__(*e); self.a.__exit__(*e)

        cn, cf = [int(v) for v in lens_h[-1]], [int(v) for v in lens_h[fl]]
        transforms = data_dict.get('transform')
        if transforms is not None:
            transforms = (torch.stack(list(transforms)) if isinstance(transforms, (list, tuple)) else transforms).reshape(B, 4, 4).contiguous()
        gt = None
        fork()
        with on(0):
            _, node_masks, knn_idx, knn_masks = GF.point_to_node_partition_batched(points_f, points_c, cf, cn, K)
            if transforms is not None:
                _, _, all_pts = GF.gather_patches_batched(None, 0, cn, cf, knn_idx, knn_masks, points_f)
                gt = GF.node_correspondences_batched(points_c, all_pts, node_masks, knn_masks, cn, transforms, self.matching_radius)

        feats = data_dict['features']
        feats_list = native.backbone_forward(feats, data_dict) if native is not None else self.backbone(feats, data_dict)
        feats_c, feats_f = feats_list[-1], feats_list[0]
        mark('backbone')

        tr = self.transformer
        emb_mod = tr.embedding
        rows_c = [int(v) for v in lens_h[-1]]
        n2 = [r * r for r in rows_c]
        eo = [0]
        for v in n2:
            eo.append(eo[-1] + v)
        C = tr.in_proj.out_features
        d_all = GF.scratch((eo[-1],), dev, 'gse_d_all')
        a_all = GF.scratch((eo[-1], emb_mod.angle_k), dev, 'gse_a_all')
        E_all = GF.scratch((eo[-1], C), dev, 'gse_E_all')
        GF.gse_indices_batched(points_c, rows_c, emb_mod.sigma_d, emb_mod.sigma_a, emb_mod.angle_k, d_all, a_all)
        wd_t = emb_mod._cache.get('wd_t', emb_mod.proj_d.weight, lambda w: w.t().contiguous())
        wa_t = emb_mod._cache.get('wa_t', emb_mod.proj_a.weight, lambda w: w.t().contiguous())
        GF.gse_embed_flat(d_all, a_all, eo[-1], emb_mod.embedding.div_term, emb_mod.proj_d.weight.detach(), emb_mod.proj_a.weight.detach(),
                          emb_mod.proj_d.bias.detach(), emb_mod.proj_a.bias.detach(), wd_t, wa_t, E_all, table=emb_mod.table())
        embs = [E_all[eo[c]:eo[c + 1]] for c in range(2 * B)]
        mark('structure_embedding')
        x = GF.linear(feats_c, tr.in_proj.weight, tr.in_proj.bias)
        if native is not None:
            x = native.transformer_forward_batched(x, rows_c, embs)
        else:
            x = tr.transformer.forward_stacked(x, rows_c[0], embs[0], embs[1])
        y = GF.linear(x, tr.out_proj.weight, tr.out_proj.bias)
        y_n = GF.l2_normalize(y)
        mark('transformer')

        join()
        mark('join_grouping+gt')
        cm, fm = self.coarse_matching, self.fine_matching
        if forced is None:
            kc = cm.num_correspondences
            corr, node_scores, corr_count = GF.superpoint_matching_batched(y_n, node_masks, cn, kc, cm.dual_normalization)
        else:
            corr, node_scores = forced
            kc = corr.shape[1]
            corr_count = torch.full((1,), kc, dtype=torch.int32, device=dev)
        k_idx, k_masks, k_pts = GF.gather_patches_batched(corr, kc, cn, cf, knn_idx, knn_masks, points_f)
        r, s = slice(0, B * kc), slice(B * kc, 2 * B * kc)
        raw_scores = GF.patch_scores_batched(feats_f, cf, k_idx[r], k_idx[s])
        scores = self.optimal_transport(raw_scores, k_masks[r], k_masks[s])
        rc, sc, cs, T, n_corr = GF.local_global_registration_batched(
            B, k_pts[r], k_pts[s], k_masks[r], k_masks[s], scores, fm.k, fm.acceptance_radius, fm.mutual, fm.confidence_threshold,
            fm.correspondence_threshold, fm.num_refinement_steps, transform_out=results if no_sync else None)
        if no_sync:
            if gt is not None and evaluator is not None:
                GF.evaluate_batched(gt[0], gt[1], gt[2], corr, corr_count, rc, sc, n_corr, transforms, results, points0,
                                    cn, [int(v) for v in lens_h[0]], evaluator.mode, evaluator.acceptance_overlap, evaluator.acceptance_radius,
                                    results[:, 16:], evaluator.acceptance_rmse, evaluator.acceptance_rre, evaluator.acceptance_rte)
            else:
                results[:, 22].copy_(n_corr)
        if ransac is not None and ransac_out is not None:
            write_ransac_rows(ransac, sc, rc, n_corr, ransac_out)
            if gt is not None and evaluator is not None:
                GF.evaluate_batched(gt[0], gt[1], gt[2], corr, corr_count, rc, sc, n_corr, transforms, ransac_out, points0,
                                    cn, [int(v) for v in lens_h[0]], evaluator.mode, evaluator.acceptance_overlap, evaluator.acceptance_radius,
                                    ransac_out[:, 18:26], evaluator.acceptance_rmse, evaluator.acceptance_rre, evaluator.acceptance_rte)
        if gt is not None and loss_func is not None and loss_out is not None:
            loss_func.write_batched(y_n, cn, gt, k_pts[r], k_pts[s], k_masks[r], k_masks[s], scores, transforms, corr_count, loss_out)
        mark('matching+sinkhorn+lgr+metrics')
        if taps is not None:
            nr = cn[0]
            taps.update(ref_node_masks=node_masks[:nr], src_node_masks=node_masks[nr:], ref_node_knn_indices=knn_idx[:nr],
                        src_node_knn_indices=knn_idx[nr:], ref_node_knn_masks=knn_masks[:nr], src_node_knn_masks=knn_masks[nr:],
                        feats_c=feats_c, feats_f=feats_f, matching_scores_raw=raw_scores)
        if no_sync:
            if not keep_outputs:
                return None
            T = T[:, :16].clone()
        outs = []
        g0 = 0
        for p in range(B):
            pr, ps = slice(p * kc, (p + 1) * kc), slice((B + p) * kc, (B + p + 1) * kc)
            o = dict(ref_points_c=cloud(points_c, oc, p), src_points_c=cloud(points_c, oc, B + p), ref_points_f=cloud(points_f, of, p),
                     src_points_f=cloud(points_f, of, B + p), ref_points=cloud(points0, o0, p), src_points=cloud(points0, o0, B + p),
                     ref_feats_c=cloud(y_n, oc, p), src_feats_c=cloud(y_n, oc, B + p), ref_feats_f=cloud(feats_f, of, p),
                     src_feats_f=cloud(feats_f, of, B + p), ref_node_corr_indices=corr[p], src_node_corr_indices=corr[B + p],
                     node_corr_scores=node_scores[p], ref_node_corr_knn_points=k_pts[pr], src_node_corr_knn_points=k_pts[ps],
                     ref_node_corr_knn_masks=k_masks[pr], src_node_corr_knn_masks=k_masks[ps], matching_scores=scores[pr],
                     ref_corr_points=rc[p], src_corr_points=sc[p], corr_scores=cs[p], estimated_transform=T[p, :16].reshape(4, 4),
                     _counts=dict(node_corr=corr_count[p], corr=n_corr[p], gt=None if gt is None else gt[2][p]))
            if gt is not None:
                g1 = g0 + cn[p] * cn[B + p]
                o['gt_node_corr_indices'], o['gt_node_corr_overlaps'] = gt[0][g0:g1], gt[1][g0:g1]
                g0 = g1
            outs.append(o)
        if no_sync:
            return outs
        main.synchronize()
        return trim_outputs(outs)

    def forward(self, data_dict, taps=None):
        outs = self.forward_batch(data_dict, taps=taps)
        return outs[0] if int(data_dict.get('batch_size', 1)) == 1 else outs


def enable_native(model):
    from .native import NativeModel
    model._native = NativeModel(model)
    if not getattr(model, '_native_hook', False):
        def _rebuild(module, incompatible_keys):
            if getattr(module, '_native', None) is not None:
                module._native = NativeModel(module)
        model.register_load_state_dict_post_hook(_rebuild)
        model._native_hook = True
    return model


def create_model(cfg):
    return GeoTransformer(cfg)


def _forced_node_corr(forced, device):
    ref, src, scores = forced
    for t, dtype, name in ((ref, torch.int64, 'ref indices'), (src, torch.int64, 'src indices'), (scores, torch.float32, 'scores')):
        if t.ndim != 1 or t.dtype != dtype or t.device != device:
            raise ValueError(f'forced_node_corr: the {name} must be a 1-D {dtype} tensor on {device}')
    if not ref.shape[0] == src.shape[0] == scores.shape[0]:
        raise ValueError('forced_node_corr: the ref indices, src indices and scores must have the same length')
    return torch.stack([ref, src]), scores.reshape(1, -1)


def trim_outputs(outs):
    for o in outs:
        cnt = o.pop('_counts')
        kk, c = int(cnt['node_corr'].item()), int(cnt['corr'].item())
        for key in ('ref_node_corr_indices', 'src_node_corr_indices', 'node_corr_scores', 'ref_node_corr_knn_points',
                    'src_node_corr_knn_points', 'ref_node_corr_knn_masks', 'src_node_corr_knn_masks', 'matching_scores'):
            o[key] = o[key][:kk]
        for key in ('ref_corr_points', 'src_corr_points', 'corr_scores'):
            o[key] = o[key][:c]
        if cnt['gt'] is not None:
            g = int(cnt['gt'].item())
            o['gt_node_corr_indices'], o['gt_node_corr_overlaps'] = o['gt_node_corr_indices'][:g], o['gt_node_corr_overlaps'][:g]
    return outs


def write_ransac_rows(ransac, src_corr_points, ref_corr_points, num_corr, out):
    rr = GF.ransac_correspondences_batched(src_corr_points, ref_corr_points, ransac.distance_threshold, ransac.num_points,
                                           ransac.num_iterations, seed=ransac.get('seed', 0), num_corr=num_corr)
    B = out.shape[0]
    out[:, :16].copy_(rr['transform'].reshape(B, 16))
    out[:, 16].copy_(rr['fitness'])
    out[:, 17].copy_(rr['inlier_rmse'])
    return rr
```

geotransformer_b200/native.py:

```python
import ctypes

import torch

from . import _lib as L
from . import functional as GF

MAX_STAGES = 6
P, I64, I32, F32 = ctypes.c_void_p, ctypes.c_int64, ctypes.c_int32, ctypes.c_float


class LinearT(ctypes.Structure):
    _fields_ = [('weight', P), ('bias', P), ('c_in', I64), ('c_out', I64), ('weight_img', P)]


class NormT(ctypes.Structure):
    _fields_ = [('gamma', P), ('beta', P)]


class KPConvT(ctypes.Structure):
    _fields_ = [('weights', P), ('weights_t', P), ('bias', P), ('kernel_points', P), ('c_in', I64), ('c_out', I64), ('sigma', F32),
                ('weights_img', P)]


class ResBlockT(ctypes.Structure):
    _fields_ = [('has_unary1', I32), ('has_shortcut', I32), ('strided', I32), ('reserved', I32), ('c_in', I64),
                ('unary1', LinearT), ('norm1', NormT), ('conv', KPConvT), ('norm_conv', NormT), ('unary2', LinearT), ('norm2', NormT),
                ('shortcut', LinearT), ('norm_sc', NormT)]


class BackboneT(ctypes.Structure):
    _fields_ = [('num_stages', I32), ('finest_decoder', I32), ('groups', I32), ('init_dim', I32), ('conv1', KPConvT), ('norm1', NormT),
                ('blocks', ResBlockT * (1 + 3 * (MAX_STAGES - 1))), ('decoders', LinearT * MAX_STAGES), ('decoder_norms', NormT * MAX_STAGES)]


class TLayerT(ctypes.Structure):
    _fields_ = [('is_self', I32), ('reserved', I32), ('w_qkv', P), ('b_qkv', P), ('w_q', P), ('b_q', P), ('w_kv', P), ('b_kv', P),
                ('wp_t', P), ('bp', P), ('att_linear', LinearT), ('att_norm', NormT), ('expand', LinearT), ('squeeze', LinearT),
                ('out_norm', NormT), ('w_qkv_img', P), ('w_q_img', P), ('w_kv_img', P)]


def _ptr(t):
    return None if t is None else t.data_ptr()


class NativeModel:

    def __init__(self, model):
        self.model = model
        self._keep = []
        self.device = next(model.parameters()).device
        self.backbone = self._build_backbone(model.backbone)
        self.layers, self.num_layers = self._build_transformer(model.transformer.transformer)
        self.hidden = model.transformer.in_proj.out_features
        self.heads = model.transformer.transformer.layers[0].attention.attention.num_heads

    def _img(self, w):
        img = GF.split_tf32(w.detach())
        self._keep.append(img)
        return _ptr(img)

    def _lin(self, mlp):
        return LinearT(_ptr(mlp.weight), _ptr(mlp.bias), mlp.in_features, mlp.out_features, self._img(mlp.weight))

    def _norm(self, gn):
        return NormT(_ptr(gn.norm.weight), _ptr(gn.norm.bias))

    def _kp(self, kp):
        w = kp.weights.detach()
        wt = w.reshape(-1, w.shape[2]).t().contiguous() if w.shape[1] % 32 == 0 else None
        if wt is not None:
            self._keep.append(wt)
        return KPConvT(_ptr(w), _ptr(wt), _ptr(kp.bias), _ptr(kp.kernel_points), w.shape[1], w.shape[2], float(kp.sigma),
                       None if wt is None else self._img(wt))

    def _res(self, blk):
        r = ResBlockT()
        r.c_in, r.strided = blk.in_channels, int(blk.strided)
        r.has_unary1 = int(not isinstance(blk.unary1, torch.nn.Identity))
        if r.has_unary1:
            r.unary1, r.norm1 = self._lin(blk.unary1.mlp), self._norm(blk.unary1.norm)
        r.conv, r.norm_conv = self._kp(blk.KPConv), self._norm(blk.norm_conv)
        r.unary2, r.norm2 = self._lin(blk.unary2.mlp), self._norm(blk.unary2.norm)
        r.has_shortcut = int(not isinstance(blk.unary_shortcut, torch.nn.Identity))
        if r.has_shortcut:
            r.shortcut, r.norm_sc = self._lin(blk.unary_shortcut.mlp), self._norm(blk.unary_shortcut.norm)
        return r

    def _build_backbone(self, bb):
        b = BackboneT()
        b.num_stages, b.finest_decoder = bb.num_stages, bb.finest_decoder
        b.groups = bb.encoder1_1.norm.num_groups
        b.init_dim = bb.encoder1_1.out_channels
        b.conv1, b.norm1 = self._kp(bb.encoder1_1.KPConv), self._norm(bb.encoder1_1.norm)
        b.blocks[0] = self._res(bb.encoder1_2)
        i = 1
        for lvl in range(2, bb.num_stages + 1):
            for j in (1, 2, 3):
                b.blocks[i] = self._res(getattr(bb, f'encoder{lvl}_{j}'))
                i += 1
        for d, lvl in enumerate(range(bb.num_stages - 1, bb.finest_decoder - 1, -1)):
            dec = getattr(bb, f'decoder{lvl}')
            b.decoders[d] = self._lin(dec.mlp)
            if lvl != bb.finest_decoder:
                b.decoder_norms[d] = self._norm(dec.norm)
        self._dec_channels = [getattr(bb, f'decoder{lvl}').mlp.out_features
                              for lvl in range(bb.num_stages - 1, bb.finest_decoder - 1, -1)]
        self._coarse_channels = getattr(bb, f'encoder{bb.num_stages}_3').out_channels
        return b

    def _build_transformer(self, tr):
        arr = (TLayerT * len(tr.layers))()
        for i, (blk, layer) in enumerate(zip(tr.blocks, tr.layers)):
            mha = layer.attention.attention
            t = TLayerT()
            t.is_self = int(blk == 'self')
            cat = lambda names, attr: torch.cat([getattr(getattr(mha, n), attr).detach() for n in names], dim=0).contiguous()
            if t.is_self:
                wqkv, bqkv = cat(('proj_q', 'proj_k', 'proj_v'), 'weight'), cat(('proj_q', 'proj_k', 'proj_v'), 'bias')
                wpt = mha.proj_p.weight.detach().t().contiguous()
                self._keep += [wqkv, bqkv, wpt]
                t.w_qkv, t.b_qkv, t.wp_t, t.bp = _ptr(wqkv), _ptr(bqkv), _ptr(wpt), _ptr(mha.proj_p.bias)
                t.w_qkv_img = self._img(wqkv)
            else:
                wkv, bkv = cat(('proj_k', 'proj_v'), 'weight'), cat(('proj_k', 'proj_v'), 'bias')
                self._keep += [wkv, bkv]
                t.w_q, t.b_q, t.w_kv, t.b_kv = _ptr(mha.proj_q.weight), _ptr(mha.proj_q.bias), _ptr(wkv), _ptr(bkv)
                t.w_q_img, t.w_kv_img = self._img(mha.proj_q.weight), self._img(wkv)
            att, ffn = layer.attention, layer.output
            t.att_linear = self._lin(att.linear)
            t.att_norm = NormT(_ptr(att.norm.weight), _ptr(att.norm.bias))
            t.expand, t.squeeze = self._lin(ffn.expand), self._lin(ffn.squeeze)
            t.out_norm = NormT(_ptr(ffn.norm.weight), _ptr(ffn.norm.bias))
            arr[i] = t
        return arr, len(tr.layers)

    def backbone_forward(self, feats, data_dict):
        lib = L.lib()
        S = self.backbone.num_stages
        pts, nb, sub, up = data_dict['points'], data_dict['neighbors'], data_dict['subsampling'], data_dict['upsampling']
        dev = feats.device
        rows = (I64 * S)(*[p.shape[0] for p in pts])
        parr = (P * S)(*[p.data_ptr() for p in pts])
        narr, nw = (P * S)(*[t.data_ptr() for t in nb]), (I64 * S)(*[t.shape[1] for t in nb])
        sarr, sw = (P * S)(*[t.data_ptr() for t in sub]), (I64 * S)(*[t.shape[1] for t in sub])
        uarr, uw = (P * S)(*[t.data_ptr() for t in up]), (I64 * S)(*[t.shape[1] for t in up])
        outs = [torch.empty((pts[-1].shape[0], self._coarse_channels), dtype=torch.float32, device=dev)]
        for d, lvl in enumerate(range(S - 1, self.backbone.finest_decoder - 1, -1)):
            outs.append(torch.empty((pts[lvl - 1].shape[0], self._dec_channels[d]), dtype=torch.float32, device=dev))
        oarr = (P * len(outs))(*[o.data_ptr() for o in outs])
        ws_bytes = lib.geob200_backbone_workspace_bytes(ctypes.byref(self.backbone), rows)
        ws = L.workspace(ws_bytes, dev, 'native_backbone')
        n_pairs = int(data_dict.get('batch_size', 1))
        gn = GF._gn_workspace(dev, self.backbone.groups, pts[0].shape[0], self.backbone.init_dim << S, n_pairs=n_pairs)
        carr = marr = None
        if n_pairs > 1:
            lens = data_dict['lengths_host']
            keep = [(I64 * (2 * n_pairs))(*[int(v) for v in lens[l]]) for l in range(S)]
            carr = (P * S)(*[ctypes.cast(k, P).value for k in keep])
            cmax = torch.empty((S - 1, 2 * n_pairs), dtype=torch.int32, device=dev)
            for l in range(S - 1):
                L.check(lib.geob200_cloud_max_count(sub[l].data_ptr(), sub[l].shape[0], pts[l].shape[0], sub[l].shape[1], n_pairs, keep[l + 1],
                                                    cmax[l].data_ptr(), L.stream_ptr()), 'cloud_max_count')
            marr = (P * S)(*([cmax[l].data_ptr() for l in range(S - 1)] + [None]))
        L.check(lib.geob200_backbone_forward_batched(ctypes.byref(self.backbone), feats.data_ptr(), parr, rows, narr, nw, sarr, sw, uarr, uw,
                                                     oarr, gn.data_ptr(), gn.numel(), ws.data_ptr(), ws.numel(), L.stream_ptr(), n_pairs, carr,
                                                     marr), 'backbone_forward_batched')
        outs.reverse()
        return outs

    def transformer_forward_batched(self, x, cloud_rows, embeddings):
        lib = L.lib()
        nc = len(cloud_rows)
        rows = (I64 * nc)(*[int(r) for r in cloud_rows])
        earr = (P * nc)(*[e.data_ptr() for e in embeddings])
        out = torch.empty_like(x)
        ws_bytes = lib.geob200_transformer_batched_workspace_bytes(nc // 2, rows, self.hidden, self.heads, self.num_layers)
        ws = L.workspace(ws_bytes, x.device, 'native_transformer')
        L.check(lib.geob200_transformer_forward_batched(self.layers, self.num_layers, self.hidden, self.heads, x.data_ptr(), nc // 2, rows,
                                                        earr, out.data_ptr(), ws.data_ptr(), ws.numel(), L.stream_ptr()),
                'transformer_forward_batched')
        return out
```

include/geob200.h:

```cpp
#ifndef GEOB200_H
#define GEOB200_H

#include <stddef.h>
#include <stdint.h>

#ifdef __cplusplus
extern "C" {
#endif

const char* geob200_last_error(void);
uint64_t geob200_launch_count(void);


size_t geob200_grid_subsample_workspace_bytes(int64_t n_points, int64_t batch);
int geob200_grid_subsample(const float* points, int64_t n_points, const int64_t* lengths_h, int64_t batch, float voxel,
                           float* s_points, int64_t* s_lengths, void* workspace, size_t workspace_bytes, void* stream);

size_t geob200_radius_search_workspace_bytes(int64_t n_query, int64_t n_support, int64_t batch);
int geob200_radius_search(const float* q_points, int64_t n_query, const float* s_points, int64_t n_support,
                          const int64_t* q_lengths_h, const int64_t* s_lengths_h, int64_t batch, float radius,
                          int64_t width, int64_t* out, int32_t* counts, int32_t* max_count, void* workspace,
                          size_t workspace_bytes, void* stream);

int geob200_neighbor_histogram(const int64_t* neighbors, int64_t n_rows, int64_t width, int64_t n_support, int64_t hist_n,
                               int32_t* hist, void* stream);


size_t geob200_kpconv_workspace_bytes(int64_t n_support);
int geob200_kpconv(const float* s_feats, const float* q_points, const float* s_points, const int64_t* neighbors,
                   int64_t n_query, int64_t n_support, int64_t n_neighbors, const float* kernel_points, int64_t n_kernel,
                   const float* weights, const float* bias, int64_t c_in, int64_t c_out, float sigma, float* out,
                   void* workspace, size_t workspace_bytes, void* stream);

size_t geob200_kpconv_tc_workspace_bytes(int64_t n_query, int64_t n_support, int64_t c_in);
int geob200_kpconv_tc(const float* s_feats, const float* q_points, const float* s_points, const int64_t* neighbors, int64_t n_query,
                      int64_t n_support, int64_t n_neighbors, const float* kernel_points, int64_t n_kernel, const float* weights_t,
                      const float* bias, int64_t c_in, int64_t c_out, float sigma, float* out, void* workspace, size_t workspace_bytes,
                      void* stream);

int geob200_split_tf32(const float* w, int64_t ld, int64_t n, int64_t k, float* out, void* stream);

void geob200_set_linear_mode(int mode);
int geob200_linear(const float* x, int64_t ldx, const float* weight, const float* bias, float* y, int64_t ldy, int64_t m,
                   int64_t n, int64_t k, int relu, void* stream);
int geob200_linear_batched(const float* x, int64_t ldx, int64_t stride_x, const float* weight, int64_t ldw, int64_t stride_w,
                           const float* bias, int64_t stride_b, float* y, int64_t ldy, int64_t stride_y, int64_t m, int64_t n,
                           int64_t k, int64_t batch, int relu, void* stream);

size_t geob200_group_norm_workspace_bytes(int64_t groups);
int geob200_group_norm(const float* x, int64_t n_rows, int64_t channels, int64_t groups, const float* gamma,
                       const float* beta, float eps, const float* residual, int leaky, float slope, float* y,
                       void* workspace, size_t workspace_bytes, void* stream);

size_t geob200_fused_group_norm_workspace_bytes(int64_t n_rows, int64_t channels, int64_t groups);
int geob200_linear_group_norm(const float* x, int64_t ldx, const float* weight, const float* bias, int64_t m, int64_t n, int64_t k,
                              int64_t groups, const float* gamma, const float* beta, float eps, const float* residual, int leaky,
                              float slope, float* pre_norm, float* y, void* workspace, size_t workspace_bytes, void* stream);
int geob200_kpconv_group_norm(const float* s_feats, const float* q_points, const float* s_points, const int64_t* neighbors,
                              int64_t n_query, int64_t n_support, int64_t n_neighbors, const float* kernel_points, int64_t n_kernel,
                              const float* weights_t, const float* bias, int64_t c_in, int64_t c_out, float sigma, int64_t groups,
                              const float* gamma, const float* beta, float eps, int leaky, float slope, float* pre_norm, float* y,
                              void* gn_workspace, size_t gn_workspace_bytes, void* workspace, size_t workspace_bytes, void* stream);

int geob200_group_norm_batched(const float* x, int64_t n_rows, int64_t channels, int64_t groups, const float* gamma, const float* beta,
                               float eps, const float* residual, int leaky, float slope, float* y, void* workspace, size_t workspace_bytes,
                               void* stream, int64_t n_pairs, const int64_t* cloud_rows_h);
int geob200_linear_group_norm_batched(const float* x, int64_t ldx, const float* weight, const float* bias, int64_t m, int64_t n, int64_t k,
                                      int64_t groups, const float* gamma, const float* beta, float eps, const float* residual, int leaky,
                                      float slope, float* pre_norm, float* y, void* workspace, size_t workspace_bytes, void* stream,
                                      int64_t n_pairs, const int64_t* cloud_rows_h);

int geob200_maxpool(const float* x, const int64_t* neighbors, int64_t n_query, int64_t n_support, int64_t n_neighbors,
                    int64_t channels, float* y, void* stream);

int geob200_cloud_max_count(const int64_t* neighbors, int64_t n_query, int64_t n_support, int64_t n_neighbors, int64_t n_pairs,
                            const int64_t* cloud_rows_h, int32_t* cloud_max, void* stream);

int geob200_upsample_concat(const float* x, const int64_t* up_indices, int64_t up_stride, int64_t n_support,
                            const float* skip, int64_t n_query, int64_t c1, int64_t c2, float* y, void* stream);


size_t geob200_kpconv_backward_workspace_bytes(int64_t n_query, int64_t n_support, int64_t n_neighbors, int64_t c_in, int64_t c_out);
int geob200_kpconv_backward(const float* s_feats, const float* q_points, const float* s_points, const int64_t* neighbors, int64_t n_query,
                            int64_t n_support, int64_t n_neighbors, const float* kernel_points, int64_t n_kernel, const float* weights,
                            int64_t c_in, int64_t c_out, float sigma, const float* grad_out, float* grad_feats, float* grad_weights,
                            float* grad_bias, void* workspace, size_t workspace_bytes, void* stream);

size_t geob200_linear_backward_workspace_bytes(int64_t m, int64_t n, int64_t k, int relu);
int geob200_linear_backward(const float* x, int64_t ldx, const float* weight_t, const float* relu_y, int64_t m, int64_t n, int64_t k,
                            const float* grad_y, float* grad_x, float* grad_weight, float* grad_bias, void* workspace, size_t workspace_bytes,
                            void* stream);

size_t geob200_group_norm_backward_batched_workspace_bytes(int64_t n_rows, int64_t channels, int64_t groups, int64_t n_pairs);
int geob200_group_norm_backward_batched(const float* x, const float* y, int64_t n_rows, int64_t channels, int64_t groups, const float* gamma,
                                        float eps, int leaky, float slope, const float* grad_y, float* grad_x, float* grad_gamma,
                                        float* grad_beta, float* grad_residual, void* workspace, size_t workspace_bytes, void* stream,
                                        int64_t n_pairs, const int64_t* cloud_rows_h);

size_t geob200_maxpool_backward_batched_workspace_bytes(int64_t n_query, int64_t n_support, int64_t n_neighbors, int64_t channels);
int geob200_maxpool_backward_batched(const float* x, const int64_t* neighbors, int64_t n_query, int64_t n_support, int64_t n_neighbors,
                                     int64_t channels, const int32_t* cloud_max, int64_t n_pairs, const int64_t* cloud_rows_h,
                                     const float* grad_y, float* grad_x, void* workspace, size_t workspace_bytes, void* stream);

size_t geob200_upsample_concat_backward_workspace_bytes(int64_t n_query, int64_t n_support);
int geob200_upsample_concat_backward(const int64_t* up_indices, int64_t up_stride, int64_t n_query, int64_t n_support, int64_t c1, int64_t c2,
                                     const float* grad_y, float* grad_x, float* grad_skip, void* workspace, size_t workspace_bytes,
                                     void* stream);


int geob200_point_to_node_partition_batched(const float* points, const float* nodes, int64_t n_clouds, const int64_t* cloud_points,
                                            const int64_t* cloud_nodes, int64_t point_limit, int64_t* point_to_node, uint8_t* node_masks,
                                            int32_t* node_sizes, int64_t* node_knn_indices, uint8_t* node_knn_masks, void* stream);

int geob200_knn_partition(const float* points, int64_t n_points, const float* nodes, int64_t n_nodes, int64_t k,
                          int64_t* knn_indices, float* knn_sq_distances, void* stream);
int geob200_pairwise_distance(const float* x, int64_t n, const float* y, int64_t m, int64_t channels, int normalized, float* out,
                              void* stream);
int geob200_point_to_node_indices(const float* points, int64_t n_points, const float* nodes, int64_t n_nodes, int64_t* indices,
                                  int32_t* node_sizes, void* stream);
int geob200_apply_transform(const float* points, int64_t n_points, const float* transform, float* out, void* stream);

int geob200_gather_rows(const float* table, int64_t n_rows, int64_t channels, const int64_t* indices, int64_t n_indices,
                        float* out, void* stream);


int geob200_gse_indices_batched(const float* points, int64_t n_clouds, const int64_t* cloud_rows_h, float sigma_d, float factor_a,
                                int64_t angle_k, float* d_indices, float* a_indices, void* stream);

size_t geob200_gse_embed_workspace_bytes(int64_t n, int64_t channels);
int geob200_gse_embed_pairs(const float* d_indices, const float* a_indices, int64_t n_rows, int64_t channels, const float* div_term,
                            const float* wd_t, const float* wa_t, const float* wd, const float* wa, const float* bd, const float* ba,
                            float* embeddings, int mode, void* workspace, size_t workspace_bytes, void* stream);

size_t geob200_gse_table_bytes(int64_t channels, int64_t inv_step, float d_max, float a_max);
int geob200_gse_table_build(const float* div_term, const float* wd_t, const float* wa_t, const float* bd, const float* ba,
                            int64_t channels, int64_t inv_step, float d_max, float a_max, void* table, size_t table_bytes,
                            void* stream);
int geob200_gse_embed_table(const float* d_indices, const float* a_indices, int64_t n_rows, int64_t channels, const void* table,
                            size_t table_bytes, int64_t inv_step, float d_max, float a_max, const float* div_term, const float* wd,
                            const float* wa, const float* bd, const float* ba, float* embeddings, void* stream);

size_t geob200_attention_workspace_bytes(int64_t n_query, int64_t n_key, int64_t heads);
int geob200_attention(const float* q, int64_t ldq, const float* k, int64_t ldk, const float* v, int64_t ldv, const float* qp,
                      const float* qb, const float* embed, int64_t n_query, int64_t n_key, int64_t channels, int64_t heads,
                      float* out, int64_t ldo, void* workspace, size_t workspace_bytes, void* stream);
typedef struct { const float* q; const float* k; const float* v; const float* qp; const float* qb; const float* embed; float* out;
                 int64_t n_query, n_key; } geob200_att_item_t;
size_t geob200_attention_batched_workspace_bytes(const geob200_att_item_t* items_h, int64_t n_items, int64_t heads);
int geob200_attention_batched(const geob200_att_item_t* items_h, int64_t n_items, int64_t ldq, int64_t ldk, int64_t ldv, int64_t ldo,
                              int64_t channels, int64_t heads, void* workspace, size_t workspace_bytes, void* stream);
int geob200_set_attention_tma(int on);
int geob200_head_bias(const float* q, int64_t ldq, const float* bias_p, int64_t n, int64_t channels, int64_t heads, float* qb,
                      void* stream);
int geob200_add_layernorm(const float* a, const float* b, const float* gamma, const float* beta, int64_t n, int64_t channels,
                          float eps, float* y, void* stream);
int geob200_l2_normalize(const float* x, int64_t n, int64_t channels, float* y, void* stream);


size_t geob200_add_layernorm_backward_workspace_bytes(int64_t n, int64_t channels);
int geob200_add_layernorm_backward(const float* a, const float* b, const float* gamma, int64_t n, int64_t channels, float eps,
                                   const float* grad_y, float* grad_x, float* grad_gamma, float* grad_beta, void* workspace,
                                   size_t workspace_bytes, void* stream);
int geob200_l2_normalize_backward(const float* x, int64_t n, int64_t channels, const float* grad_y, float* grad_x, void* stream);
size_t geob200_head_project_backward_workspace_bytes(int64_t n, int64_t channels, int64_t heads);
int geob200_head_project_backward(const float* q, int64_t ldq, const float* wp, const float* bp, int64_t n, int64_t channels, int64_t heads,
                                  const float* grad_qp, const float* grad_qb, float* grad_q, int64_t ldgq, float* grad_wp, float* grad_bp,
                                  void* workspace, size_t workspace_bytes, void* stream);
typedef struct { const float* probs; const float* grad_out; float* grad_q; float* grad_k; float* grad_v; float* grad_qp; float* grad_qb;
                 float* grad_embed; } geob200_att_grad_item_t;
size_t geob200_attention_backward_batched_workspace_bytes(const geob200_att_item_t* items_h, int64_t n_items, int64_t heads);
int geob200_attention_backward_batched(const geob200_att_item_t* items_h, const geob200_att_grad_item_t* grads_h, int64_t n_items,
                                       int64_t ldq, int64_t ldk, int64_t ldv, int64_t ldo, int64_t ldgq, int64_t ldgk, int64_t ldgv,
                                       int64_t channels, int64_t heads, void* workspace, size_t workspace_bytes, void* stream);
size_t geob200_gse_embed_backward_workspace_bytes(int64_t n_rows, int64_t channels);
int geob200_gse_embed_backward(const float* d_indices, const float* a_indices, int64_t n_rows, int64_t angle_k, int64_t channels,
                               const void* table, size_t table_bytes, int64_t inv_step, float d_max, float a_max, const float* div_term,
                               const float* wa, const float* ba, const float* grad_embed, float* grad_wd, float* grad_bd, float* grad_wa,
                               float* grad_ba, void* workspace, size_t workspace_bytes, void* stream);


size_t geob200_superpoint_matching_batched_workspace_bytes(int64_t n_rows, int64_t n_products, int64_t n_pairs);
int geob200_superpoint_matching_batched(const float* ref_feats, const float* src_feats, int64_t channels, const uint8_t* ref_masks,
                                        const uint8_t* src_masks, int64_t n_pairs, const int64_t* cloud_nodes, int64_t num_correspondences,
                                        int dual, int64_t* corr_indices, float* corr_scores, int32_t* num_out, void* workspace,
                                        size_t workspace_bytes, void* stream);

int geob200_gather_patches_batched(const int64_t* corr_indices, int64_t n_corr, int64_t n_clouds, const int64_t* cloud_nodes,
                                   const int64_t* cloud_points, const int64_t* node_knn_indices, const uint8_t* node_knn_masks, int64_t k,
                                   const float* points, int64_t* out_indices, uint8_t* out_masks, float* out_points, void* stream);

int geob200_patch_scores_batched(const float* ref_feats, const float* src_feats, int64_t channels, int64_t n_pairs, const int64_t* cloud_points,
                                 const int64_t* ref_knn_indices, const int64_t* src_knn_indices, int64_t n_patches, int64_t k,
                                 float* scores, void* stream);

size_t geob200_patch_scores_backward_batched_workspace_bytes(int64_t n_rows, int64_t n_patches_total, int64_t k, int64_t channels);
int geob200_patch_scores_backward_batched(const float* ref_feats, const float* src_feats, int64_t channels, int64_t n_pairs,
                                          const int64_t* cloud_points, const int64_t* ref_knn_indices, const int64_t* src_knn_indices,
                                          int64_t n_patches, int64_t k, const float* grad_scores, float* grad_ref_feats,
                                          float* grad_src_feats, void* workspace, size_t workspace_bytes, void* stream);

int geob200_sinkhorn(const float* scores, const uint8_t* row_masks, const uint8_t* col_masks, const float* alpha,
                     int64_t n_patches, int64_t k, int64_t num_iterations, float inf, float* out, void* stream);

size_t geob200_sinkhorn_backward_workspace_bytes(int64_t n_patches, int64_t k, int64_t num_iterations);
int geob200_sinkhorn_backward(const float* scores, const uint8_t* row_masks, const uint8_t* col_masks, const float* alpha, int64_t n_patches,
                              int64_t k, int64_t num_iterations, float inf, const float* grad_out, float* grad_scores, float* grad_alpha,
                              void* workspace, size_t workspace_bytes, void* stream);


size_t geob200_lgr_batched_workspace_bytes(int64_t n_pairs, int64_t n_patches, int64_t k, int64_t topk);
int geob200_local_global_registration_batched(const float* ref_knn_points, const float* src_knn_points, const uint8_t* ref_knn_masks,
                                              const uint8_t* src_knn_masks, const float* log_scores, int64_t n_pairs, int64_t n_patches,
                                              int64_t k, int64_t score_ld, int64_t topk, float acceptance_radius, int mutual,
                                              float confidence_threshold, int64_t correspondence_threshold, int64_t num_refinement_steps,
                                              float* ref_corr_points, float* src_corr_points, float* corr_scores, int32_t* corr_patch,
                                              int32_t* num_corr, float* estimated_transform, int64_t transform_ld, float* patch_transforms,
                                              int32_t* patch_inliers, int32_t* best_patch, void* workspace, size_t workspace_bytes,
                                              void* stream);

int geob200_weighted_procrustes(const float* src_points, const float* ref_points, const float* weights, int64_t batch,
                                int64_t n, float weight_thresh, float eps, float* transforms, void* stream);

size_t geob200_node_correspondences_batched_workspace_bytes(int64_t n_rows, int64_t n_products, int64_t k);
int geob200_node_correspondences_batched(const float* ref_nodes, const float* src_nodes, const float* ref_knn_points,
                                         const float* src_knn_points, const uint8_t* ref_masks, const uint8_t* src_masks,
                                         const uint8_t* ref_knn_masks, const uint8_t* src_knn_masks, int64_t n_pairs, const int64_t* cloud_nodes,
                                         int64_t k, const float* transforms, float pos_radius, int64_t* corr_indices, float* corr_overlaps,
                                         int32_t* count, void* workspace, size_t workspace_bytes, void* stream);

int geob200_evaluate_counts(const int64_t* gt_node_corr_indices, const float* gt_node_corr_overlaps, int64_t n_gt, const int32_t* n_gt_dev,
                            float acceptance_overlap, const int64_t* ref_node_corr_indices, const int64_t* src_node_corr_indices,
                            int64_t n_node_corr, const int32_t* n_node_corr_dev, const float* ref_corr_points, const float* src_corr_points,
                            int64_t n_corr, const int32_t* n_corr_dev, float acceptance_radius, const float* gt_transform,
                            const float* est_transform, const float* src_points, int64_t n_src_points, int mode, float rmse_threshold,
                            float rre_threshold, float rte_threshold, float* metrics, void* stream);
int geob200_evaluate_batched(const int64_t* gt_node_corr_indices, const float* gt_node_corr_overlaps, const int32_t* n_gt_dev,
                             float acceptance_overlap, const int64_t* ref_node_corr_indices, const int64_t* src_node_corr_indices,
                             int64_t n_node_corr, const int32_t* n_node_corr_dev, const float* ref_corr_points, const float* src_corr_points,
                             int64_t n_corr, const int32_t* n_corr_dev, float acceptance_radius, const float* gt_transforms,
                             const float* est_transforms, int64_t transform_ld, const float* points, int64_t n_pairs, const int64_t* cloud_nodes,
                             const int64_t* cloud_points, int mode, float rmse_threshold, float rre_threshold, float rte_threshold,
                             float* metrics, int64_t metrics_ld, void* stream);

size_t geob200_coarse_matching_loss_batched_workspace_bytes(int64_t n_rows, int64_t n_products);
int geob200_coarse_matching_loss_batched(const float* ref_feats, const float* src_feats, int64_t channels, int64_t n_pairs,
                                         const int64_t* cloud_nodes, const int64_t* gt_node_corr_indices, const float* gt_node_corr_overlaps,
                                         const int32_t* gt_count, float positive_margin, float negative_margin, float positive_optimal,
                                         float negative_optimal, float log_scale, float positive_overlap, float* out, int64_t out_ld,
                                         void* workspace, size_t workspace_bytes, void* stream);
size_t geob200_fine_matching_loss_batched_workspace_bytes(int64_t n_pairs, int64_t n_patches);
int geob200_fine_matching_loss_batched(const float* ref_knn_points, const float* src_knn_points, const uint8_t* ref_knn_masks,
                                       const uint8_t* src_knn_masks, const float* matching_scores, const float* transforms, int64_t n_pairs,
                                       int64_t n_patches, int64_t k, const int32_t* patch_count, double positive_radius,
                                       const float* loss_weights, float* out, int64_t out_ld, void* workspace, size_t workspace_bytes,
                                       void* stream);

size_t geob200_coarse_matching_loss_backward_batched_workspace_bytes(int64_t n_rows, int64_t n_products, int64_t n_pairs);
int geob200_coarse_matching_loss_backward_batched(const float* ref_feats, const float* src_feats, int64_t channels, int64_t n_pairs,
                                                  const int64_t* cloud_nodes, const int64_t* gt_node_corr_indices,
                                                  const float* gt_node_corr_overlaps, const int32_t* gt_count, float positive_margin,
                                                  float negative_margin, float positive_optimal, float negative_optimal, float log_scale,
                                                  float positive_overlap, const float* grad_rows, int64_t grad_ld, const float* loss_weights,
                                                  float* grad_ref_feats, float* grad_src_feats, void* workspace, size_t workspace_bytes,
                                                  void* stream);
size_t geob200_fine_matching_loss_backward_batched_workspace_bytes(int64_t n_pairs, int64_t n_patches);
int geob200_fine_matching_loss_backward_batched(const float* ref_knn_points, const float* src_knn_points, const uint8_t* ref_knn_masks,
                                                const uint8_t* src_knn_masks, const float* transforms, int64_t n_pairs, int64_t n_patches,
                                                int64_t k, const int32_t* patch_count, double positive_radius, const float* grad_rows,
                                                int64_t grad_ld, const float* loss_weights, float* grad_scores, void* workspace,
                                                size_t workspace_bytes, void* stream);

size_t geob200_ransac_correspondences_batched_workspace_bytes(int64_t n_pairs, int64_t num_iterations);
int geob200_ransac_correspondences_batched(const float* ref_corr_points, const float* src_corr_points, int64_t n_pairs, int64_t capacity,
                                           const int32_t* num_corr, float distance_threshold, int64_t ransac_n, int64_t num_iterations,
                                           uint64_t seed, int64_t pair_base, float* transforms, float* fitness, float* inlier_rmse,
                                           int32_t* inlier_count,
                                           int32_t* best_iteration, float* hyp_transforms, int32_t* hyp_inliers, float* hyp_rmse,
                                           int32_t* hyp_samples, void* workspace, size_t workspace_bytes, void* stream);

size_t geob200_correspondence_metrics_batched_workspace_bytes(int64_t n_pairs, int64_t capacity);
int geob200_correspondence_metrics_batched(const float* ref_corr_points, const float* src_corr_points, int64_t n_pairs, int64_t capacity,
                                           const int32_t* num_corr, const float* transforms, int64_t transform_ld, float positive_radius,
                                           float* out, int64_t out_ld, void* workspace, size_t workspace_bytes, void* stream);

size_t geob200_feature_nn_batched_workspace_bytes(int64_t n_pairs, int64_t cap_query, int64_t cap_support);
int geob200_feature_nn_batched(const float* query, const float* support, int64_t n_pairs, int64_t cap_query, int64_t cap_support,
                               int64_t channels, const int32_t* n_query, const int32_t* n_support, int64_t* query_index,
                               double* query_dist, int64_t* support_index, double* support_dist, void* workspace, size_t workspace_bytes,
                               void* stream);
int geob200_feature_corr_indices(const int64_t* ref_nn, const double* ref_dist, const int64_t* src_nn, const double* src_dist,
                                 int64_t n_ref, int64_t n_src, int32_t mode, int64_t* ref_corr, int64_t* src_corr, float* feat_dist,
                                 int32_t* count, void* stream);
size_t geob200_ransac_features_batched_workspace_bytes(int64_t n_pairs, int64_t cap_src, int64_t cap_ref, int64_t num_iterations,
                                                       int64_t val_iterations);
int geob200_ransac_features_batched(const float* src_points, const float* ref_points, const float* src_feats, const float* ref_feats,
                                    int64_t n_pairs, int64_t cap_src, int64_t cap_ref, int64_t channels, const int32_t* n_src,
                                    const int32_t* n_ref, float distance_threshold, int64_t ransac_n, int64_t num_iterations,
                                    int64_t val_iterations, uint64_t seed, int64_t pair_base, float* transforms, float* fitness,
                                    float* inlier_rmse, int32_t* inlier_count, int32_t* best_iteration, int32_t* num_validated,
                                    int64_t* rec_matches, int32_t* rec_samples, int32_t* rec_pass, int32_t* rec_val_ids,
                                    float* rec_transforms, int32_t* rec_inliers, float* rec_rmse, void* workspace, size_t workspace_bytes,
                                    void* stream);

int geob200_corr_order_batched(const float* scores, int64_t n_pairs, int64_t capacity, const int32_t* num_corr, int64_t kmax, int32_t* order,
                               void* stream);
int geob200_corr_select_batched(const float* ref_corr_points, const float* src_corr_points, const float* corr_scores, int64_t n_pairs,
                                int64_t capacity, const int32_t* num_corr, const int32_t* order, int64_t kmax, int64_t k,
                                float* ref_out, float* src_out, float* scores_out, int32_t* count_out, void* stream);
size_t geob200_sparse_correspondence_eval_batched_workspace_bytes(int64_t n_pairs, int64_t m_cap, int64_t n_cap);
int geob200_sparse_correspondence_eval_batched(const int64_t* ref_node_corr_indices, const int64_t* src_node_corr_indices, int64_t pred_cap,
                                               const int32_t* pred_count, const int64_t* gt_node_corr_indices, int64_t gt_cap,
                                               const int32_t* gt_count, int64_t n_pairs, int64_t m_cap, int64_t n_cap, double* out,
                                               void* workspace, size_t workspace_bytes, void* stream);
int geob200_registration_error_batched(const float* gt_transforms, int64_t gt_ld, const float* est_transforms, int64_t est_ld,
                                       const float* covariances, const int32_t* has_covariance, int64_t n_pairs, int mode,
                                       double threshold0, double threshold1, double* out, void* stream);
int geob200_weighted_procrustes_counts(const float* src_points, const float* ref_points, const float* weights, int64_t batch,
                                       int64_t capacity, const int32_t* counts, float weight_thresh, float eps, float* transforms,
                                       void* stream);

int geob200_linear_profile_enable(int on);
int geob200_set_split_k(int on);
int geob200_set_linear_persistent(int on);
int64_t geob200_linear_profile_read(int64_t capacity, int64_t* shapes, float* ms);

#define GEOB200_MAX_STAGES 6
typedef struct { const float* weight; const float* bias; int64_t c_in, c_out; const float* weight_img; } geob200_linear_t;
typedef struct { const float* gamma; const float* beta; } geob200_norm_t;
typedef struct { const float* weights; const float* weights_t; const float* bias; const float* kernel_points;
                 int64_t c_in, c_out; float sigma; const float* weights_img; } geob200_kpconv_t;
typedef struct {
    int32_t has_unary1, has_shortcut, strided, reserved;
    int64_t c_in;
    geob200_linear_t unary1; geob200_norm_t norm1;
    geob200_kpconv_t conv;   geob200_norm_t norm_conv;
    geob200_linear_t unary2; geob200_norm_t norm2;
    geob200_linear_t shortcut; geob200_norm_t norm_sc;
} geob200_resblock_t;
typedef struct {
    int32_t num_stages, finest_decoder, groups, init_dim;
    geob200_kpconv_t conv1; geob200_norm_t norm1;
    geob200_resblock_t blocks[1 + 3 * (GEOB200_MAX_STAGES - 1)];
    geob200_linear_t decoders[GEOB200_MAX_STAGES];
    geob200_norm_t decoder_norms[GEOB200_MAX_STAGES];
} geob200_backbone_t;
size_t geob200_backbone_workspace_bytes(const geob200_backbone_t* net, const int64_t* level_rows);
int geob200_backbone_forward_batched(const geob200_backbone_t* net, const float* feats, const float* const* points,
                                     const int64_t* level_rows, const int64_t* const* neighbors, const int64_t* neighbor_width,
                                     const int64_t* const* subsampling, const int64_t* subsampling_width,
                                     const int64_t* const* upsampling, const int64_t* upsampling_width, float* const* out_feats,
                                     void* gn_workspace, size_t gn_workspace_bytes, void* workspace, size_t workspace_bytes, void* stream,
                                     int64_t n_pairs, const int64_t* const* cloud_rows_h, const int32_t* const* sub_cloud_max);

typedef struct {
    int32_t is_self, reserved;
    const float* w_qkv; const float* b_qkv; const float* w_q; const float* b_q; const float* w_kv; const float* b_kv;
    const float* wp_t; const float* bp;
    geob200_linear_t att_linear; geob200_norm_t att_norm;
    geob200_linear_t expand; geob200_linear_t squeeze; geob200_norm_t out_norm;
    const float* w_qkv_img; const float* w_q_img; const float* w_kv_img;
} geob200_tlayer_t;
size_t geob200_transformer_batched_workspace_bytes(int64_t n_pairs, const int64_t* cloud_rows_h, int64_t channels, int64_t heads,
                                                   int64_t num_layers);
int geob200_transformer_forward_batched(const geob200_tlayer_t* layers, int64_t num_layers, int64_t channels, int64_t heads,
                                        const float* x, int64_t n_pairs, const int64_t* cloud_rows_h, const float* const* embeddings_h,
                                        float* out, void* workspace, size_t workspace_bytes, void* stream);

#ifdef __cplusplus
}
#endif
#endif
```

Measured before the change: 428.5.

## Fuse geometric structure embedding generation into first self-attention score kernel

The first self-attention layer now computes the geometric structure embedding rows from the table lookup inside the attention scoring kernel. Each row is written out with streaming stores for later layers and dotted with the projected queries at the same time. This removes the separate embedding kernel and the extra read of the large N×N×C embedding tensor during the first layer's scoring. In exchange, the new persistent kernel does table interpolation per key inside attention, and the host plumbing grows with new struct and event handling.

```diff
diff --git a/geotransformer_b200/_lib.py b/geotransformer_b200/_lib.py
--- a/geotransformer_b200/_lib.py
+++ b/geotransformer_b200/_lib.py
@@ -135,9 +135,10 @@
 _sig('geob200_backbone_forward_batched', c_int, P, P, P, P, P, P, P, P, P, P, P, P, SZ, P, SZ, P, I64, P, P)
 _sig('geob200_cloud_max_count', c_int, P, I64, I64, I64, I64, P, P, P)
 _sig('geob200_transformer_batched_workspace_bytes', SZ, I64, P, I64, I64, I64)
-_sig('geob200_transformer_forward_batched', c_int, P, I64, I64, I64, P, I64, P, P, P, P, SZ, P)
+_sig('geob200_transformer_forward_batched', c_int, P, I64, I64, I64, P, I64, P, P, P, P, SZ, P, P)
 _sig('geob200_attention_batched_workspace_bytes', SZ, P, I64, I64)
 _sig('geob200_attention_batched', c_int, P, I64, I64, I64, I64, I64, I64, I64, P, SZ, P)
+_sig('geob200_attention_embed_batched', c_int, P, I64, I64, I64, I64, I64, I64, I64, P, P, P, SZ, I64, F, F, P, P, P, P, P, P, SZ, P)
 
 
 def lib():
diff --git a/geotransformer_b200/csrc/attention.cu b/geotransformer_b200/csrc/attention.cu
--- a/geotransformer_b200/csrc/attention.cu
+++ b/geotransformer_b200/csrc/attention.cu
@@ -1,6 +1,7 @@
 #include "attention.cuh"
 #include "common.cuh"
 #include "geob200.h"
+#include "gse_table.cuh"
 
 namespace geob200 {
 
@@ -418,7 +419,8 @@
 }
 
 static int attention_streaming_batch(const geob200_att_item_t* items, int64_t n_items, int64_t ldq, int64_t ldk, int64_t ldv, int64_t ldo,
-                                     int64_t channels, int64_t heads, void* workspace, size_t workspace_bytes, cudaStream_t st) {
+                                     int64_t channels, int64_t heads, void* workspace, size_t workspace_bytes, cudaStream_t st,
+                                     const AttEmbedSrc* gse = nullptr) {
     if (!(channels == 128 || channels == 256) || workspace == nullptr) return 1;
     GEOB_REQUIRE(n_items >= 1 && n_items <= ATT_MAX_ITEMS, "attention: 1..%d items per launch", ATT_MAX_ITEMS);
     AttBatch b{};
@@ -446,6 +448,11 @@
     }
     GEOB_REQUIRE(workspace_bytes >= need, "attention: workspace too small");
     const float div = sqrtf((float)(channels / heads));
+    if (gse != nullptr) {
+        const int rt = attention_tma_embed_batch(b, *gse, (int)ldq, (int)ldk, (int)ldv, (int)ldo, (int)channels, (int)heads, div, st);
+        GEOB_REQUIRE(rt != 1, "attention_embed: unsupported shape (channels %lld, heads %lld)", (long long)channels, (long long)heads);
+        return rt;
+    }
     if (g_att_tma) {
         const int rt = attention_tma_batch(b, (int)ldq, (int)ldk, (int)ldv, (int)ldo, (int)channels, (int)heads, div, st);
         if (rt <= 0) return rt;
@@ -508,6 +515,58 @@
     return 0;
 }
 
+}
+
+namespace geob200 {
+int attention_embed_batched(const geob200_att_item_t* items, int64_t n_items, int64_t ldq, int64_t ldk, int64_t ldv, int64_t ldo,
+                            int64_t channels, int64_t heads, const float* const* d_indices, const float* const* a_indices,
+                            const void* table, size_t table_bytes, int64_t inv_step, float d_max, float a_max, const float* div_term,
+                            const float* wd, const float* wa, const float* bd, const float* ba, void* workspace, size_t workspace_bytes,
+                            void* stream, void* ev_begin, void* ev_end) {
+    cudaStream_t st = (cudaStream_t)stream;
+    if (n_items == 0) return 0;
+    if (attention_check(channels, heads, ldq, ldk, ldv)) return -2;
+    GEOB_REQUIRE(channels == 128 || channels == 256, "attention_embed: channels %lld unsupported (128 or 256)", (long long)channels);
+    GEOB_REQUIRE(workspace != nullptr, "attention_embed: needs the workspace of geob200_attention_batched_workspace_bytes");
+    GEOB_REQUIRE(inv_step >= 1 && (inv_step & (inv_step - 1)) == 0, "attention_embed: inv_step must be a power of two");
+    GEOB_REQUIRE(table_bytes >= geob200_gse_table_bytes(channels, inv_step, d_max, a_max) && table_bytes > 0,
+                 "attention_embed: table buffer smaller than (channels, inv_step, d_max, a_max) imply");
+    GEOB_REQUIRE(((uintptr_t)table & 15) == 0, "attention_embed: table must be 16-byte aligned");
+    AttEmbedSrc g{};
+    g.table = (const unsigned char*)table;
+    g.div_term = div_term; g.wd = wd; g.wa = wa; g.bd = bd; g.ba = ba;
+    g.n_d = gtab::node_count(d_max, (int)inv_step);
+    g.n_a = gtab::node_count(a_max, (int)inv_step);
+    g.inv_step = (float)inv_step;
+    for (int64_t i0 = 0; i0 < n_items; i0 += ATT_MAX_ITEMS) {
+        const int64_t cnt = (n_items - i0 < ATT_MAX_ITEMS) ? n_items - i0 : ATT_MAX_ITEMS;
+        for (int64_t i = 0; i < cnt; ++i) {
+            const geob200_att_item_t& it = items[i0 + i];
+            GEOB_REQUIRE(it.embed != nullptr && it.n_query == it.n_key && d_indices[i0 + i] != nullptr && a_indices[i0 + i] != nullptr,
+                         "attention_embed: item %lld needs embed, its indices and n_query == n_key", (long long)(i0 + i));
+            g.d[i] = d_indices[i0 + i];
+            g.a[i] = a_indices[i0 + i];
+        }
+        g.ev_begin = i0 == 0 ? (cudaEvent_t)ev_begin : nullptr;
+        g.ev_end = i0 + cnt == n_items ? (cudaEvent_t)ev_end : nullptr;
+        const int rc = attention_streaming_batch(items + i0, cnt, ldq, ldk, ldv, ldo, channels, heads, workspace, workspace_bytes, st, &g);
+        if (rc != 0) return rc;
+    }
+    return 0;
+}
+}
+
+extern "C" {
+
+int geob200_attention_embed_batched(const geob200_att_item_t* items, int64_t n_items, int64_t ldq, int64_t ldk, int64_t ldv, int64_t ldo,
+                                    int64_t channels, int64_t heads, const float* const* d_indices, const float* const* a_indices,
+                                    const void* table, size_t table_bytes, int64_t inv_step, float d_max, float a_max, const float* div_term,
+                                    const float* wd, const float* wa, const float* bd, const float* ba, void* workspace,
+                                    size_t workspace_bytes, void* stream) {
+    return attention_embed_batched(items, n_items, ldq, ldk, ldv, ldo, channels, heads, d_indices, a_indices, table, table_bytes, inv_step,
+                                   d_max, a_max, div_term, wd, wa, bd, ba, workspace, workspace_bytes, stream, nullptr, nullptr);
+}
+
 int geob200_attention(const float* q, int64_t ldq, const float* k, int64_t ldk, const float* v, int64_t ldv, const float* qp,
                       const float* qb, const float* embed, int64_t n_query, int64_t n_key, int64_t channels, int64_t heads,
                       float* out, int64_t ldo, void* workspace, size_t workspace_bytes, void* stream) {
diff --git a/geotransformer_b200/csrc/attention.cuh b/geotransformer_b200/csrc/attention.cuh
--- a/geotransformer_b200/csrc/attention.cuh
+++ b/geotransformer_b200/csrc/attention.cuh
@@ -1,5 +1,7 @@
 #pragma once
 #include <cuda_runtime.h>
+
+#include "geob200.h"
 
 namespace geob200 {
 
@@ -13,6 +15,24 @@
     AttItem it[ATT_MAX_ITEMS];
 };
 
+struct AttEmbedSrc {
+    const float* d[ATT_MAX_ITEMS];
+    const float* a[ATT_MAX_ITEMS];
+    const unsigned char* table;
+    const float *div_term, *wd, *wa, *bd, *ba;
+    int n_d, n_a;
+    float inv_step;
+    cudaEvent_t ev_begin, ev_end;
+};
+
 int attention_tma_batch(const AttBatch& b, int ldq, int ldk, int ldv, int ldo, int channels, int heads, float div, cudaStream_t st);
+int attention_tma_embed_batch(const AttBatch& b, const AttEmbedSrc& g, int ldq, int ldk, int ldv, int ldo, int channels, int heads,
+                              float div, cudaStream_t st);
+
+int attention_embed_batched(const geob200_att_item_t* items, int64_t n_items, int64_t ldq, int64_t ldk, int64_t ldv, int64_t ldo,
+                            int64_t channels, int64_t heads, const float* const* d_indices, const float* const* a_indices,
+                            const void* table, size_t table_bytes, int64_t inv_step, float d_max, float a_max, const float* div_term,
+                            const float* wd, const float* wa, const float* bd, const float* ba, void* workspace, size_t workspace_bytes,
+                            void* stream, void* ev_begin, void* ev_end);
 
 }
diff --git a/geotransformer_b200/csrc/attention_tma.cu b/geotransformer_b200/csrc/attention_tma.cu
--- a/geotransformer_b200/csrc/attention_tma.cu
+++ b/geotransformer_b200/csrc/attention_tma.cu
@@ -1,6 +1,7 @@
 #include "attention.cuh"
 #include "common.cuh"
 #include "geob200.h"
+#include "gse_table.cuh"
 
 namespace geob200 {
 
@@ -187,6 +188,96 @@
             for (int m = lane; m < M; m += 32) dst[m] = sh[m] / sum;
         }
         asm volatile("bar.sync 1, %0;" ::"n"(ATM_CW * 32) : "memory");
+    }
+}
+
+constexpr int ATE_W = ATM_KCH;
+constexpr int ATE_THREADS = ATE_W * 32;
+constexpr int ATE_CTAS = 2;
+
+template <int H, int J>
+__global__ void __launch_bounds__(ATE_THREADS, ATE_CTAS) att_stream_embed_kernel(const __grid_constant__ AttBatch b,
+                                                                                 const __grid_constant__ AttEmbedSrc g, float div, int max_m) {
+    using LK = gtab::Lookup<128 * J>;
+    constexpr int C = 128 * J;
+    static_assert(H == 1 || H == 2 || H == 4 || H == 8, "heads must be 1, 2, 4 or 8");
+    extern __shared__ float4 ate_smem[];
+    const int mp = (max_m + 3) & ~3;
+    float4* idx = ate_smem;
+    float4* qps = idx + mp;
+    float* sc = reinterpret_cast<float*>(qps + H * (C / 4));
+    const int warp = threadIdx.x >> 5, lane = threadIdx.x & 31;
+    const float scale = reinterpret_cast<const gtab::Header*>(g.table)->slope_scale;
+    const unsigned char* __restrict__ td = g.table + gtab::HEADER_BYTES;
+    const unsigned char* __restrict__ ta = td + (size_t)g.n_d * LK::NODE;
+    const float lim_d = (float)g.n_d, lim_a = (float)g.n_a;
+    const long long units = b.uprefix[b.n_items];
+    const long long u_begin = units * blockIdx.x / gridDim.x, u_end = units * (blockIdx.x + 1) / gridDim.x;
+    constexpr int KG = 8 / H, NV = KG * H;
+    constexpr int SH = 2;
+    const int vidx = lane >> SH, vu = vidx / H, vh = vidx % H;
+    const bool lead = (lane & ((1 << SH) - 1)) == 0;
+    int ci = 0;
+    for (long long u = u_begin; u < u_end; ++u) {
+        while (u >= b.uprefix[ci + 1]) ++ci;
+        const AttItem& it = b.it[ci];
+        const int M = it.M;
+        const int n = (int)(u - b.uprefix[ci]);
+        const long long r0 = (long long)n * M;
+        for (int m = threadIdx.x; m < M; m += ATE_THREADS) {
+            const float* a = g.a[ci] + 3 * (r0 + m);
+            idx[m] = make_float4(g.d[ci][r0 + m], a[0], a[1], a[2]);
+        }
+        for (int t = threadIdx.x; t < H * (C / 4); t += ATE_THREADS)
+            qps[t] = reinterpret_cast<const float4*>(it.qp + (long long)n * H * C)[t];
+        const float qb_h = it.qb[(long long)n * H + vh];
+        float* S_row = it.S + ((long long)n * H + vh) * M;
+        float4* __restrict__ E = reinterpret_cast<float4*>(const_cast<float*>(it.E) + r0 * C);
+        __syncthreads();
+        for (int m0 = 0; m0 < M; m0 += ATE_W * KG) {
+            const int mk = m0 + warp + ATE_W * vu;
+            const bool writer = lead && mk < M;
+            const float sqk = writer ? S_row[mk] : 0.f;
+            float v[NV];
+#pragma unroll
+            for (int u = 0; u < KG; ++u) {
+                const int m = m0 + warp + ATE_W * u;
+#pragma unroll
+                for (int h = 0; h < H; ++h) v[u * H + h] = 0.f;
+                if (m < M) {
+                    const typename LK::Row e = LK::row(idx[m], td, ta, lim_d, lim_a, g.inv_step, scale, g.div_term, g.wd, g.wa, g.bd, g.ba, lane);
+#pragma unroll
+                    for (int j = 0; j < J; ++j) {
+                        const float4 x = make_float4(e.v[4 * j + 0], e.v[4 * j + 1], e.v[4 * j + 2], e.v[4 * j + 3]);
+                        __stcs(E + (long long)m * (C / 4) + j * 32 + lane, x);
+#pragma unroll
+                        for (int h = 0; h < H; ++h) {
+                            const float4 q = qps[h * (C / 4) + j * 32 + lane];
+                            v[u * H + h] = fmaf(x.x, q.x, fmaf(x.y, q.y, fmaf(x.z, q.z, fmaf(x.w, q.w, v[u * H + h]))));
+                        }
+                    }
+                }
+            }
+            warp_butterfly(v, lane);
+            if (writer) sc[vh * mp + mk] = (sqk + v[0] + qb_h) / div;
+        }
+        __syncthreads();
+        for (int h = warp; h < H; h += ATE_W) {
+            float* sh = sc + h * mp;
+            float mx = -INFINITY;
+            for (int m = lane; m < M; m += 32) mx = fmaxf(mx, sh[m]);
+            mx = warp_max(mx);
+            float sum = 0.f;
+            for (int m = lane; m < M; m += 32) {
+                const float e = expf(sh[m] - mx);
+                sh[m] = e;
+                sum += e;
+            }
+            sum = warp_sum(sum);
+            float* dst = it.S + ((long long)n * H + h) * M;
+            for (int m = lane; m < M; m += 32) dst[m] = sh[m] / sum;
+        }
+        __syncthreads();
     }
 }
 
@@ -301,6 +392,51 @@
     return 0;
 }
 
+template <int H, int J>
+static int launch_tma_embed(const AttBatch& b, const AttEmbedSrc& g, int ldq, int ldk, int ldv, int ldo, int max_n, int max_m, size_t smem,
+                            float div, cudaStream_t st) {
+    constexpr int C = 128 * J, D = C / H;
+    const dim3 qk_grid((unsigned)((max_m + ATQ_T - 1) / ATQ_T), (unsigned)((max_n + ATQ_T - 1) / ATQ_T), (unsigned)(b.n_items * H));
+    att_qk_kernel<H><<<qk_grid, 256, 0, st>>>(b, ldq, ldk, D);
+    if (smem > 48 * 1024 && ensure_max_smem((const void*)att_stream_embed_kernel<H, J>)) return -1;
+    int occ = 0;
+    if (cudaOccupancyMaxActiveBlocksPerMultiprocessor(&occ, att_stream_embed_kernel<H, J>, ATE_THREADS, smem) != cudaSuccess || occ < 1) occ = 1;
+    const long long units = b.uprefix[b.n_items];
+    long long grid = (long long)occ * num_sms();
+    if (grid > units) grid = units;
+    if (g.ev_begin != nullptr) GEOB_CHECK_CUDA(cudaEventRecord(g.ev_begin, st));
+    att_stream_embed_kernel<H, J><<<(unsigned)grid, ATE_THREADS, smem, st>>>(b, g, div, max_m);
+    if (g.ev_end != nullptr) GEOB_CHECK_CUDA(cudaEventRecord(g.ev_end, st));
+    const dim3 pv_grid((unsigned)((max_n + ATQ_T - 1) / ATQ_T), (unsigned)(H * ((D + 63) / 64)), (unsigned)b.n_items);
+    att_pv_kernel<H><<<pv_grid, 256, 0, st>>>(b, ldv, ldo, D);
+    return 0;
+}
+
+int attention_tma_embed_batch(const AttBatch& b, const AttEmbedSrc& g, int ldq, int ldk, int ldv, int ldo, int channels, int heads,
+                              float div, cudaStream_t st) {
+    if (!(channels == 128 || channels == 256)) return 1;
+    int max_n = 0, max_m = 0;
+    for (int i = 0; i < b.n_items; ++i) { max_n = b.it[i].N > max_n ? b.it[i].N : max_n; max_m = b.it[i].M > max_m ? b.it[i].M : max_m; }
+    const size_t smem = (size_t)((max_m + 3) & ~3) * (16 + sizeof(float) * heads) + sizeof(float) * heads * channels;
+    if (smem > 200 * 1024) return 1;
+    int rc = -2;
+#define LAUNCH_EMBED(HV) \
+    rc = (channels == 256) ? launch_tma_embed<HV, 2>(b, g, ldq, ldk, ldv, ldo, max_n, max_m, smem, div, st) \
+                           : launch_tma_embed<HV, 1>(b, g, ldq, ldk, ldv, ldo, max_n, max_m, smem, div, st)
+    switch (heads) {
+        case 1: LAUNCH_EMBED(1); break;
+        case 2: LAUNCH_EMBED(2); break;
+        case 4: LAUNCH_EMBED(4); break;
+        case 8: LAUNCH_EMBED(8); break;
+        default: return 1;
+    }
+#undef LAUNCH_EMBED
+    if (rc != 0) return rc;
+    GEOB_CHECK_LAUNCH();
+    count_launches(3);
+    return 0;
+}
+
 int attention_tma_batch(const AttBatch& b, int ldq, int ldk, int ldv, int ldo, int channels, int heads, float div, cudaStream_t st) {
     if (b.it[0].E == nullptr) {
         int rc = -2;
diff --git a/geotransformer_b200/csrc/gse_table.cu b/geotransformer_b200/csrc/gse_table.cu
--- a/geotransformer_b200/csrc/gse_table.cu
+++ b/geotransformer_b200/csrc/gse_table.cu
@@ -104,30 +104,10 @@
         const long long left = n_pairs - p0;
         const int cnt = left < 32 ? (int)left : 32;
         for (int r = 0; r < cnt; ++r) {
-            const float4 x = idx_s[warp][r];
-            const float t0 = x.x * inv_step, t1 = x.y * inv_step, t2 = x.z * inv_step, t3 = x.w * inv_step;
-            const bool in0 = t0 >= 0.f && t0 < lim_d, in1 = t1 >= 0.f && t1 < lim_a, in2 = t2 >= 0.f && t2 < lim_a,
-                       in3 = t3 >= 0.f && t3 < lim_a;
-            float* __restrict__ row = E + (p0 + r) * C;
-            if (!(in0 && in1 && in2 && in3)) {
-                LK::slow_row(x, td, ta, lim_d, lim_a, inv_step, scale, div_term, Wd, Wa, bd, ba, lane, row);
-                continue;
-            }
-            float vd[4 * NV], va[4 * NV], vb[4 * NV], vc[4 * NV];
-            const int i0 = (int)t0, i1 = (int)t1, i2 = (int)t2, i3 = (int)t3;
-            LK::interp(td, i0, (t0 - (float)i0) * scale, lane, vd);
-            LK::interp(ta, i1, (t1 - (float)i1) * scale, lane, va);
-            LK::interp(ta, i2, (t2 - (float)i2) * scale, lane, vb);
-            LK::interp(ta, i3, (t3 - (float)i3) * scale, lane, vc);
+            const typename LK::Row e = LK::row(idx_s[warp][r], td, ta, lim_d, lim_a, inv_step, scale, div_term, Wd, Wa, bd, ba, lane);
+            float4* __restrict__ row = reinterpret_cast<float4*>(E + (p0 + r) * C);
 #pragma unroll
-            for (int j = 0; j < NV; ++j) {
-                float4 o;
-                o.x = vd[4 * j + 0] + fmaxf(fmaxf(va[4 * j + 0], vb[4 * j + 0]), vc[4 * j + 0]);
-                o.y = vd[4 * j + 1] + fmaxf(fmaxf(va[4 * j + 1], vb[4 * j + 1]), vc[4 * j + 1]);
-                o.z = vd[4 * j + 2] + fmaxf(fmaxf(va[4 * j + 2], vb[4 * j + 2]), vc[4 * j + 2]);
-                o.w = vd[4 * j + 3] + fmaxf(fmaxf(va[4 * j + 3], vb[4 * j + 3]), vc[4 * j + 3]);
-                __stcs(reinterpret_cast<float4*>(row) + 32 * j + lane, o);
-            }
+            for (int j = 0; j < NV; ++j) __stcs(row + 32 * j + lane, make_float4(e.v[4 * j + 0], e.v[4 * j + 1], e.v[4 * j + 2], e.v[4 * j + 3]));
         }
     }
 }
diff --git a/geotransformer_b200/csrc/gse_table.cuh b/geotransformer_b200/csrc/gse_table.cuh
--- a/geotransformer_b200/csrc/gse_table.cuh
+++ b/geotransformer_b200/csrc/gse_table.cuh
@@ -65,19 +65,23 @@
     static __device__ __forceinline__ void term(float x, const unsigned char* __restrict__ tab, float lim, float inv_step, float scale,
                                                 const float* __restrict__ div_term, const float* __restrict__ W,
                                                 const float* __restrict__ bias, int lane, float (&val)[4 * NV]) {
-        const float t = x * inv_step;
+        const float t = __fmul_rn(x, inv_step);
         if (t >= 0.f && t < lim) {
             const int i = (int)t;
-            interp(tab, i, (t - (float)i) * scale, lane, val);
+            interp(tab, i, __fmul_rn(__fsub_rn(t, (float)i), scale), lane, val);
         } else {
             exact(x, div_term, W, bias, lane, val);
         }
     }
 
-    static __device__ __noinline__ void slow_row(float4 x, const unsigned char* __restrict__ td, const unsigned char* __restrict__ ta,
-                                                 float lim_d, float lim_a, float inv_step, float scale, const float* __restrict__ div_term,
-                                                 const float* __restrict__ Wd, const float* __restrict__ Wa, const float* __restrict__ bd,
-                                                 const float* __restrict__ ba, int lane, float* __restrict__ row) {
+    struct Row {
+        float v[4 * NV];
+    };
+
+    static __device__ __noinline__ Row slow_row(float4 x, const unsigned char* __restrict__ td, const unsigned char* __restrict__ ta,
+                                                float lim_d, float lim_a, float inv_step, float scale, const float* __restrict__ div_term,
+                                                const float* __restrict__ Wd, const float* __restrict__ Wa, const float* __restrict__ bd,
+                                                const float* __restrict__ ba, int lane) {
         float acc[4 * NV], val[4 * NV];
         term(x.y, ta, lim_a, inv_step, scale, div_term, Wa, ba, lane, acc);
         term(x.z, ta, lim_a, inv_step, scale, div_term, Wa, ba, lane, val);
@@ -87,11 +91,30 @@
 #pragma unroll
         for (int q = 0; q < 4 * NV; ++q) acc[q] = fmaxf(acc[q], val[q]);
         term(x.x, td, lim_d, inv_step, scale, div_term, Wd, bd, lane, val);
+        Row r;
 #pragma unroll
-        for (int j = 0; j < NV; ++j)
-            __stcs(reinterpret_cast<float4*>(row) + 32 * j + lane,
-                   make_float4(val[4 * j + 0] + acc[4 * j + 0], val[4 * j + 1] + acc[4 * j + 1], val[4 * j + 2] + acc[4 * j + 2],
-                               val[4 * j + 3] + acc[4 * j + 3]));
+        for (int q = 0; q < 4 * NV; ++q) r.v[q] = __fadd_rn(val[q], acc[q]);
+        return r;
+    }
+
+    static __device__ __forceinline__ Row row(float4 x, const unsigned char* __restrict__ td, const unsigned char* __restrict__ ta,
+                                              float lim_d, float lim_a, float inv_step, float scale, const float* __restrict__ div_term,
+                                              const float* __restrict__ Wd, const float* __restrict__ Wa, const float* __restrict__ bd,
+                                              const float* __restrict__ ba, int lane) {
+        const float t0 = __fmul_rn(x.x, inv_step), t1 = __fmul_rn(x.y, inv_step), t2 = __fmul_rn(x.z, inv_step),
+                    t3 = __fmul_rn(x.w, inv_step);
+        const bool in0 = t0 >= 0.f && t0 < lim_d, in1 = t1 >= 0.f && t1 < lim_a, in2 = t2 >= 0.f && t2 < lim_a, in3 = t3 >= 0.f && t3 < lim_a;
+        if (!(in0 && in1 && in2 && in3)) return slow_row(x, td, ta, lim_d, lim_a, inv_step, scale, div_term, Wd, Wa, bd, ba, lane);
+        float vd[4 * NV], va[4 * NV], vb[4 * NV], vc[4 * NV];
+        const int i0 = (int)t0, i1 = (int)t1, i2 = (int)t2, i3 = (int)t3;
+        interp(td, i0, __fmul_rn(__fsub_rn(t0, (float)i0), scale), lane, vd);
+        interp(ta, i1, __fmul_rn(__fsub_rn(t1, (float)i1), scale), lane, va);
+        interp(ta, i2, __fmul_rn(__fsub_rn(t2, (float)i2), scale), lane, vb);
+        interp(ta, i3, __fmul_rn(__fsub_rn(t3, (float)i3), scale), lane, vc);
+        Row r;
+#pragma unroll
+        for (int q = 0; q < 4 * NV; ++q) r.v[q] = __fadd_rn(vd[q], fmaxf(fmaxf(va[q], vb[q]), vc[q]));
+        return r;
     }
 };
 
diff --git a/geotransformer_b200/csrc/native.cu b/geotransformer_b200/csrc/native.cu
--- a/geotransformer_b200/csrc/native.cu
+++ b/geotransformer_b200/csrc/native.cu
@@ -1,3 +1,4 @@
+#include "attention.cuh"
 #include "common.cuh"
 #include "geob200.h"
 
@@ -224,7 +225,7 @@
 
 int geob200_transformer_forward_batched(const geob200_tlayer_t* layers, int64_t num_layers, int64_t channels, int64_t heads,
                                         const float* x_in, int64_t n_pairs, const int64_t* cloud_rows_h, const float* const* embeddings,
-                                        float* out, void* workspace, size_t workspace_bytes, void* stream) {
+                                        float* out, void* workspace, size_t workspace_bytes, void* stream, const geob200_gse_src_t* gse) {
     GEOB_REQUIRE(n_pairs >= 1 && 2 * n_pairs <= GEOB_MAX_CLOUDS, "transformer: 1 <= pairs per batch <= %d", GEOB_MAX_CLOUDS / 2);
     Ctx c(workspace, workspace_bytes);
     c.stream = stream;
@@ -244,6 +245,17 @@
         if (cross > att_ws_bytes) att_ws_bytes = cross;
     }
     void* att_ws = c.fl((int64_t)(att_ws_bytes / 4 + 1), 1);
+    const float* d_idx[GEOB_MAX_CLOUDS];
+    const float* a_idx[GEOB_MAX_CLOUDS];
+    if (gse != nullptr) {
+        int64_t r = 0;
+        for (int64_t cl = 0; cl < NC; ++cl) {
+            d_idx[cl] = gse->d_indices + r;
+            a_idx[cl] = gse->a_indices + 3 * r;
+            r += cloud_rows_h[cl] * cloud_rows_h[cl];
+        }
+    }
+    bool embed_pending = gse != nullptr;
     for (int64_t i = 0; i < num_layers; ++i) {
         const geob200_tlayer_t& L = layers[i];
         float* y = (i == num_layers - 1) ? out : c.fl(n, C);
@@ -262,7 +274,14 @@
                 items[cl] = geob200_att_item_t{qkv + o * 3 * C, qkv + o * 3 * C + C, qkv + o * 3 * C + 2 * C, qp + o * H * C, qb + o * H,
                                                embeddings[cl], hidden + o * C, cloud_rows_h[cl], cloud_rows_h[cl]};
             }
-            TRY(geob200_attention_batched(items, NC, 3 * C, 3 * C, 3 * C, C, C, H, att_ws, att_ws_bytes, stream));
+            if (embed_pending) {
+                TRY(attention_embed_batched(items, NC, 3 * C, 3 * C, 3 * C, C, C, H, d_idx, a_idx, gse->table, gse->table_bytes, gse->inv_step,
+                                            gse->d_max, gse->a_max, gse->div_term, gse->wd, gse->wa, gse->bd, gse->ba, att_ws, att_ws_bytes,
+                                            stream, gse->event_begin, gse->event_end));
+                embed_pending = false;
+            } else {
+                TRY(geob200_attention_batched(items, NC, 3 * C, 3 * C, 3 * C, C, C, H, att_ws, att_ws_bytes, stream));
+            }
             TRY(run_tail(c, L, hidden, x, n, C, y));
         } else {
             const int64_t Sn = n - R;
diff --git a/geotransformer_b200/model.py b/geotransformer_b200/model.py
--- a/geotransformer_b200/model.py
+++ b/geotransformer_b200/model.py
@@ -120,15 +120,19 @@
         a_all = GF.scratch((eo[-1], emb_mod.angle_k), dev, 'gse_a_all')
         E_all = GF.scratch((eo[-1], C), dev, 'gse_E_all')
         GF.gse_indices_batched(points_c, rows_c, emb_mod.sigma_d, emb_mod.sigma_a, emb_mod.angle_k, d_all, a_all)
-        wd_t = emb_mod._cache.get('wd_t', emb_mod.proj_d.weight, lambda w: w.t().contiguous())
-        wa_t = emb_mod._cache.get('wa_t', emb_mod.proj_a.weight, lambda w: w.t().contiguous())
-        GF.gse_embed_flat(d_all, a_all, eo[-1], emb_mod.embedding.div_term, emb_mod.proj_d.weight.detach(), emb_mod.proj_a.weight.detach(),
-                          emb_mod.proj_d.bias.detach(), emb_mod.proj_a.bias.detach(), wd_t, wa_t, E_all, table=emb_mod.table())
+        table = emb_mod.table()
+        gse = (d_all, a_all, emb_mod, table) if native is not None and table is not None else None
+        if gse is None:
+            wd_t = emb_mod._cache.get('wd_t', emb_mod.proj_d.weight, lambda w: w.t().contiguous())
+            wa_t = emb_mod._cache.get('wa_t', emb_mod.proj_a.weight, lambda w: w.t().contiguous())
+            GF.gse_embed_flat(d_all, a_all, eo[-1], emb_mod.embedding.div_term, emb_mod.proj_d.weight.detach(),
+                              emb_mod.proj_a.weight.detach(), emb_mod.proj_d.bias.detach(), emb_mod.proj_a.bias.detach(), wd_t, wa_t, E_all,
+                              table=table)
         embs = [E_all[eo[c]:eo[c + 1]] for c in range(2 * B)]
         mark('structure_embedding')
         x = GF.linear(feats_c, tr.in_proj.weight, tr.in_proj.bias)
         if native is not None:
-            x = native.transformer_forward_batched(x, rows_c, embs)
+            x = native.transformer_forward_batched(x, rows_c, embs, gse)
         else:
             x = tr.transformer.forward_stacked(x, rows_c[0], embs[0], embs[1])
         y = GF.linear(x, tr.out_proj.weight, tr.out_proj.bias)
diff --git a/geotransformer_b200/native.py b/geotransformer_b200/native.py
--- a/geotransformer_b200/native.py
+++ b/geotransformer_b200/native.py
@@ -37,6 +37,11 @@
     _fields_ = [('is_self', I32), ('reserved', I32), ('w_qkv', P), ('b_qkv', P), ('w_q', P), ('b_q', P), ('w_kv', P), ('b_kv', P),
                 ('wp_t', P), ('bp', P), ('att_linear', LinearT), ('att_norm', NormT), ('expand', LinearT), ('squeeze', LinearT),
                 ('out_norm', NormT), ('w_qkv_img', P), ('w_q_img', P), ('w_kv_img', P)]
+
+
+class GseSrcT(ctypes.Structure):
+    _fields_ = [('d_indices', P), ('a_indices', P), ('table', P), ('table_bytes', ctypes.c_size_t), ('inv_step', I64), ('d_max', F32),
+                ('a_max', F32), ('div_term', P), ('wd', P), ('wa', P), ('bd', P), ('ba', P), ('event_begin', P), ('event_end', P)]
 
 
 def _ptr(t):
@@ -168,8 +173,20 @@
         outs.reverse()
         return outs
 
-    def transformer_forward_batched(self, x, cloud_rows, embeddings):
+    def transformer_forward_batched(self, x, cloud_rows, embeddings, gse=None):
         lib = L.lib()
+        src = None
+        if gse is not None:
+            d_all, a_all, emb, tab = gse
+            src = GseSrcT(d_all.data_ptr(), a_all.data_ptr(), tab.blob.data_ptr(), tab.blob.numel(), tab.inv_step, tab.d_max, tab.a_max,
+                          emb.embedding.div_term.data_ptr(), emb.proj_d.weight.data_ptr(), emb.proj_a.weight.data_ptr(),
+                          emb.proj_d.bias.data_ptr(), emb.proj_a.bias.data_ptr(), None, None)
+            if GF.EVENTS is not None:
+                ev = (torch.cuda.Event(enable_timing=True), torch.cuda.Event(enable_timing=True))
+                for e in ev:
+                    e.record()
+                src.event_begin, src.event_end = ev[0].cuda_event, ev[1].cuda_event
+                GF.EVENTS.setdefault('gse_embed', []).append(ev)
         nc = len(cloud_rows)
         rows = (I64 * nc)(*[int(r) for r in cloud_rows])
         earr = (P * nc)(*[e.data_ptr() for e in embeddings])
@@ -177,6 +194,7 @@
         ws_bytes = lib.geob200_transformer_batched_workspace_bytes(nc // 2, rows, self.hidden, self.heads, self.num_layers)
         ws = L.workspace(ws_bytes, x.device, 'native_transformer')
         L.check(lib.geob200_transformer_forward_batched(self.layers, self.num_layers, self.hidden, self.heads, x.data_ptr(), nc // 2, rows,
-                                                        earr, out.data_ptr(), ws.data_ptr(), ws.numel(), L.stream_ptr()),
+                                                        earr, out.data_ptr(), ws.data_ptr(), ws.numel(), L.stream_ptr(),
+                                                        None if src is None else ctypes.byref(src)),
                 'transformer_forward_batched')
         return out
diff --git a/include/geob200.h b/include/geob200.h
--- a/include/geob200.h
+++ b/include/geob200.h
@@ -149,6 +149,11 @@
 size_t geob200_attention_batched_workspace_bytes(const geob200_att_item_t* items_h, int64_t n_items, int64_t heads);
 int geob200_attention_batched(const geob200_att_item_t* items_h, int64_t n_items, int64_t ldq, int64_t ldk, int64_t ldv, int64_t ldo,
                               int64_t channels, int64_t heads, void* workspace, size_t workspace_bytes, void* stream);
+int geob200_attention_embed_batched(const geob200_att_item_t* items_h, int64_t n_items, int64_t ldq, int64_t ldk, int64_t ldv, int64_t ldo,
+                                    int64_t channels, int64_t heads, const float* const* d_indices_h, const float* const* a_indices_h,
+                                    const void* table, size_t table_bytes, int64_t inv_step, float d_max, float a_max, const float* div_term,
+                                    const float* wd, const float* wa, const float* bd, const float* ba, void* workspace,
+                                    size_t workspace_bytes, void* stream);
 int geob200_set_attention_tma(int on);
 int geob200_head_bias(const float* q, int64_t ldq, const float* bias_p, int64_t n, int64_t channels, int64_t heads, float* qb,
                       void* stream);
@@ -360,11 +365,17 @@
     geob200_linear_t expand; geob200_linear_t squeeze; geob200_norm_t out_norm;
     const float* w_qkv_img; const float* w_q_img; const float* w_kv_img;
 } geob200_tlayer_t;
+typedef struct {
+    const float* d_indices; const float* a_indices;
+    const void* table; size_t table_bytes; int64_t inv_step; float d_max, a_max;
+    const float* div_term; const float* wd; const float* wa; const float* bd; const float* ba;
+    void* event_begin; void* event_end;
+} geob200_gse_src_t;
 size_t geob200_transformer_batched_workspace_bytes(int64_t n_pairs, const int64_t* cloud_rows_h, int64_t channels, int64_t heads,
                                                    int64_t num_layers);
 int geob200_transformer_forward_batched(const geob200_tlayer_t* layers, int64_t num_layers, int64_t channels, int64_t heads,
                                         const float* x, int64_t n_pairs, const int64_t* cloud_rows_h, const float* const* embeddings_h,
-                                        float* out, void* workspace, size_t workspace_bytes, void* stream);
+                                        float* out, void* workspace, size_t workspace_bytes, void* stream, const geob200_gse_src_t* gse);
 
 #ifdef __cplusplus
 }
```

After: 435.7, median of 6. About the same (+1.7%).
